# fboehm/DBSLMM

Hardware: AMD Instinct MI355X
Metric: SNPs solved/sec (whole node) + max-|Δβ| vs CPU ref, 1M SNP × 10k indiv (higher is better)
Workload: dtype f64

## Files before the change

dbslmm_amd/csrc/kernels.hip:

```cpp
#include <hip/hip_runtime.h>
#include <stdint.h>

#include "dims.hpp"

namespace {

typedef int v4i __attribute__((ext_vector_type(4)));
typedef int v16i __attribute__((ext_vector_type(16)));

constexpr int kWave = 64;
constexpr int kLdsStride = 33;

__device__ __forceinline__ void wave_sync() {
    __builtin_amdgcn_fence(__ATOMIC_RELEASE, "wavefront");
    __builtin_amdgcn_wave_barrier();
    __builtin_amdgcn_fence(__ATOMIC_ACQUIRE, "wavefront");
}

__device__ __forceinline__ int wave_sum_i32(int v) {
#pragma unroll
    for (int o = 32; o > 0; o >>= 1) v += __shfl_xor(v, o, kWave);
    return v;
}

__device__ __forceinline__ double wave_sum_f64(double v) {
#pragma unroll
    for (int o = 32; o > 0; o >>= 1) v += __shfl_xor(v, o, kWave);
    return v;
}

__device__ __forceinline__ uint32_t dose_code16(uint32_t w) {
    return 0xAAAAAAAAu - (w - ((w >> 1) & 0x55555555u));
}
__device__ __forceinline__ int64_t image_row(const int32_t* __restrict__ slot_pos, int row0, int li, int m,
                                             int32_t zrow) {
    const int32_t pos = li < m ? slot_pos[row0 + li] : -1;
    return pos < 0 ? zrow : pos;
}
typedef int v8i __attribute__((ext_vector_type(8)));
typedef float v16f __attribute__((ext_vector_type(16)));
constexpr int kE8M0Two = static_cast<int>(0x80808080u);
constexpr uint32_t kFp4Mask = 0x33333333u;
__device__ __forceinline__ v4i fp4_chunk(uint32_t w0, uint32_t w1) {
    const uint64_t t = ((static_cast<uint64_t>(w1) << 32) | w0) >> 2;
    return v4i{static_cast<int>(w0 & kFp4Mask), static_cast<int>(static_cast<uint32_t>(t) & kFp4Mask),
               static_cast<int>(w1 & kFp4Mask), static_cast<int>(static_cast<uint32_t>(t >> 32) & kFp4Mask)};
}
__device__ __forceinline__ v16f mfma_fp4(v4i a, v4i b, v16f c) {
    const v8i a8{a[0], a[1], a[2], a[3], 0, 0, 0, 0}, b8{b[0], b[1], b[2], b[3], 0, 0, 0, 0};
    return __builtin_amdgcn_mfma_scale_f32_32x32x64_f8f6f4(a8, b8, c, 4, 4, 0, kE8M0Two, 0, kE8M0Two);
}
constexpr int kE8M0Half = 0x7E7E7E7E;
__device__ __forceinline__ uint32_t raw_k44() {
    uint32_t k = 0x44444444u;
    asm volatile("" : "+v"(k));
    return k;
}
__device__ __forceinline__ v4i fp4_chunk_raw(uint32_t w0, uint32_t w1, uint32_t k44) {
    const uint64_t t = ((static_cast<uint64_t>(w1) << 32) | w0) >> 2;
    return v4i{static_cast<int>((w0 & kFp4Mask) | k44), static_cast<int>((static_cast<uint32_t>(t) & kFp4Mask) | k44),
               static_cast<int>((w1 & kFp4Mask) | k44), static_cast<int>((static_cast<uint32_t>(t >> 32) & kFp4Mask) | k44)};
}
__device__ __forceinline__ v16f mfma_fp4_raw(v4i a, v4i b, v16f c) {
    const v8i a8{a[0], a[1], a[2], a[3], 0, 0, 0, 0}, b8{b[0], b[1], b[2], b[3], 0, 0, 0, 0};
    return __builtin_amdgcn_mfma_scale_f32_32x32x64_f8f6f4(a8, b8, c, 4, 4, 0, kE8M0Half, 0, kE8M0Half);
}
__device__ __forceinline__ int gram_row(double s, int64_t kpad) { return 3 * static_cast<int>(s) - 9 * static_cast<int>(kpad); }
__device__ __forceinline__ int gram_col(double s) { return 3 * static_cast<int>(s); }
__device__ __forceinline__ int gram_exact(float t, int ri, int cj) { return static_cast<int>(t) + ri + cj; }
__device__ __forceinline__ double centre(double g, double sisj, double rn) {
    return __builtin_fma(-sisj, rn, g);
}
__device__ __forceinline__ void split_missing(uint32_t w, uint32_t& g, uint32_t& o) {
    const uint32_t m2 = w & ~(w >> 1) & 0x55555555u;
    g = dose_code16(w) & ~(3u * m2);
    o = m2 ^ 0x55555555u;
}

}

typedef unsigned int u4v __attribute__((ext_vector_type(4)));
__device__ __forceinline__ u4v load_u4(const uint8_t* p) { return *reinterpret_cast<const u4v*>(p); }
__device__ __forceinline__ u4v shift_pair(u4v x, u4v y, int d, int bs) {
    uint32_t w[8] = {x[0], x[1], x[2], x[3], y[0], y[1], y[2], y[3]};
    uint32_t o[5];
    switch (d) {
        case 0: o[0] = w[0]; o[1] = w[1]; o[2] = w[2]; o[3] = w[3]; o[4] = w[4]; break;
        case 1: o[0] = w[1]; o[1] = w[2]; o[2] = w[3]; o[3] = w[4]; o[4] = w[5]; break;
        case 2: o[0] = w[2]; o[1] = w[3]; o[2] = w[4]; o[3] = w[5]; o[4] = w[6]; break;
        default: o[0] = w[3]; o[1] = w[4]; o[2] = w[5]; o[3] = w[6]; o[4] = w[7]; break;
    }
    u4v r;
#pragma unroll
    for (int j = 0; j < 4; ++j) r[j] = __builtin_amdgcn_alignbyte(o[j + 1], o[j], static_cast<uint32_t>(bs));
    return r;
}

__device__ __forceinline__ void count_word(uint32_t word, int& sum, int& sq, int& nmiss) {
    const uint32_t lo2 = word & 0x55555555u;
    const uint32_t hi2 = (word >> 1) & 0x55555555u;
    const int n_miss = __builtin_popcount(lo2 & ~hi2);
    const int n_two = __builtin_popcount(~lo2 & ~hi2 & 0x55555555u);
    const int n_one = __builtin_popcount(~lo2 & hi2);
    nmiss += n_miss;
    sum += 2 * n_two + n_one;
    sq += 4 * n_two + n_one;
}
__device__ __forceinline__ void row_moments(int32_t n_ref, int sum, int sq, int nmiss, double& ds, double& mu,
                                            double& rsd) {
    const double dc = static_cast<double>(n_ref - nmiss);
    ds = static_cast<double>(sum);
    mu = ds / dc;
    const double css = static_cast<double>(sq) - ds * ds / dc;
    const double sd = sqrt(css / static_cast<double>(n_ref - 1));
    rsd = 1.0 / sd;
}

extern "C" __global__ __launch_bounds__(256) void dbslmm_bed_repitch(
    const uint8_t* __restrict__ bed, int32_t n_ref, int64_t bytes_per_snp, int32_t n_rows,
    uint8_t* __restrict__ img, int64_t pitch, v4i* __restrict__ tab) {
    const int lane = threadIdx.x & (kWave - 1);
    const int r = blockIdx.x * (blockDim.x / kWave) + (threadIdx.x / kWave);
    if (r > n_rows) return;
    u4v* out = reinterpret_cast<u4v*>(img + static_cast<int64_t>(r) * pitch);
    const int nq = static_cast<int>(pitch / 16);
    if (r == n_rows) {
        for (int q = lane; q < nq; q += kWave) out[q] = u4v{~0u, ~0u, ~0u, ~0u};
        if (lane == 0) tab[r] = v4i{0, 0, 0, 0};
        return;
    }
    const int64_t row_off = 3 + static_cast<int64_t>(r) * bytes_per_snp;
    const uint8_t* base = bed + (row_off & ~int64_t(15));
    const int sh = static_cast<int>(row_off & 15), dsh = sh >> 2, bsh = sh & 3;
    const int nqd = (n_ref + 63) / 64;
    int sum = 0, sq = 0, nmiss = 0;
    for (int q = lane; q < nq; q += kWave) {
        u4v g = u4v{~0u, ~0u, ~0u, ~0u};
        if (q < nqd) {
            const u4v lo = load_u4(base + 16 * static_cast<int64_t>(q));
            const u4v wv = sh ? shift_pair(lo, load_u4(base + 16 * static_cast<int64_t>(q) + 16), dsh, bsh) : lo;
#pragma unroll
            for (int j = 0; j < 4; ++j) {
                const int nv = min(16, max(0, n_ref - (64 * q + 16 * j)));
                const uint32_t keep = nv >= 16 ? ~0u : (1u << (2 * nv)) - 1u;
                g[j] = wv[j] | ~keep;
                count_word(g[j], sum, sq, nmiss);
            }
        }
        out[q] = g;
    }
    sum = wave_sum_i32(sum);
    sq = wave_sum_i32(sq);
    nmiss = wave_sum_i32(nmiss);
    if (lane == 0) tab[r] = v4i{sum, sq, nmiss, 0};
}

__device__ __forceinline__ void slot_stats_of(
    int slot, const v4i* __restrict__ tab, int32_t n_ref,
    const int32_t* __restrict__ slot_pos, const int32_t* __restrict__ slot_block, int32_t n_slots,
    double* __restrict__ S_out, double* __restrict__ mu_out, double* __restrict__ rsd_out,
    int32_t* __restrict__ block_flags) {
    if (slot >= n_slots) return;
    const int32_t pos = slot_pos ? slot_pos[slot] : slot;
    double ds = 0.0, mu = 0.0, rsd = 0.0;
    int nmiss = 0;
    if (pos >= 0) {
        const v4i e = tab[pos];
        nmiss = e[2];
        row_moments(n_ref, e[0], e[1], nmiss, ds, mu, rsd);
    }
    if (S_out) S_out[slot] = ds;
    if (mu_out) mu_out[slot] = mu;
    if (rsd_out) rsd_out[slot] = rsd;
    if (nmiss > 0 && block_flags) atomicOr(block_flags + (slot_block ? slot_block[slot] : slot), 1);
}

extern "C" __global__ __launch_bounds__(256) void dbslmm_slot_stats(
    const v4i* __restrict__ tab, int32_t n_ref,
    const int32_t* __restrict__ slot_pos, const int32_t* __restrict__ slot_block, int32_t n_slots,
    double* __restrict__ S_out, double* __restrict__ mu_out, double* __restrict__ rsd_out,
    int32_t* __restrict__ block_flags) {
    slot_stats_of(blockIdx.x * blockDim.x + threadIdx.x, tab, n_ref, slot_pos, slot_block, n_slots, S_out, mu_out,
                  rsd_out, block_flags);
}

constexpr int kFrontCopies = 4;
struct PcgFront {
    double shift[kFrontCopies];
    double* dshift;
    int32_t n;
    int32_t n_status;
    int32_t* status;
    int32_t* active;
    int32_t* next;
};
extern "C" __global__ __launch_bounds__(256) void dbslmm_pcg_front(
    const v4i* __restrict__ tab, int32_t n_ref,
    const int32_t* __restrict__ slot_pos, const int32_t* __restrict__ slot_block, int32_t n_slots,
    double* __restrict__ S_out, double* __restrict__ mu_out, double* __restrict__ rsd_out,
    int32_t* __restrict__ block_flags, PcgFront f) {
    const int t = blockIdx.x * blockDim.x + threadIdx.x, nt = gridDim.x * blockDim.x;
    for (int i = t; i < f.n_status; i += nt) f.status[i] = 0;
    if (t < f.n) f.dshift[t] = t == 0 ? f.shift[0] : t == 1 ? f.shift[1] : t == 2 ? f.shift[2] : f.shift[3];
    if (t == 0) *f.active = 0;
    if (t < 4 && f.next) f.next[t] = 0;
    slot_stats_of(t, tab, n_ref, slot_pos, slot_block, n_slots, S_out, mu_out, rsd_out, block_flags);
}

extern "C" __global__ __launch_bounds__(256) void dbslmm_snp_stats(
    const uint8_t* __restrict__ img, int32_t n_ref, int64_t pitch,
    const int32_t* __restrict__ slot_pos, int32_t n_slots,
    double* __restrict__ mu_out, double* __restrict__ rsd_out) {
    constexpr int kU = 4;
    const int lane = threadIdx.x & (kWave - 1);
    const int slot = blockIdx.x * (blockDim.x / kWave) + (threadIdx.x / kWave);
    if (slot >= n_slots) return;
    const int32_t pos = slot_pos[slot];
    if (pos < 0) {
        if (lane == 0) {
            mu_out[slot] = 0.0;
            rsd_out[slot] = 0.0;
        }
        return;
    }
    const uint8_t* base = img + static_cast<int64_t>(pos) * pitch;
    const int nqd = (n_ref + 63) / 64;
    int sum = 0, sq = 0, nmiss = 0;
    for (int q0 = 0; q0 < nqd; q0 += kWave * kU) {
        u4v wv[kU];
#pragma unroll
        for (int u = 0; u < kU; ++u) {
            const int q = q0 + kWave * u + lane;
            wv[u] = u4v{~0u, ~0u, ~0u, ~0u};
            if (q < nqd) wv[u] = load_u4(base + 16 * static_cast<int64_t>(q));
        }
#pragma unroll
        for (int u = 0; u < kU; ++u) {
#pragma unroll
            for (int j = 0; j < 4; ++j) count_word(wv[u][j], sum, sq, nmiss);
        }
    }
    sum = wave_sum_i32(sum);
    sq = wave_sum_i32(sq);
    nmiss = wave_sum_i32(nmiss);
    if (lane == 0) {
        double ds, mu, rsd;
        row_moments(n_ref, sum, sq, nmiss, ds, mu, rsd);
        mu_out[slot] = mu;
        rsd_out[slot] = rsd;
    }
}

extern "C" __global__ __launch_bounds__(256) void dbslmm_maf_arma(
    const uint8_t* __restrict__ img, int32_t n_ref, int64_t pitch,
    const int32_t* __restrict__ pos, int32_t n_rows, const double* __restrict__ mu,
    double* __restrict__ maf_out, const double* __restrict__ S, const int32_t* __restrict__ miss) {
    const int k = blockIdx.x * blockDim.x + threadIdx.x;
    if (k >= n_rows) return;
    if (miss && S && miss[k] == 0) {
        const double af = 0.5 * S[k] / static_cast<double>(n_ref);
        maf_out[k] = (1.0 - af) < af ? 1.0 - af : af;
        return;
    }
    const uint32_t* row = reinterpret_cast<const uint32_t*>(img + static_cast<int64_t>(pos ? pos[k] : k) * pitch);
    const double m = mu[k];
    double a1 = 0.0, a2 = 0.0;
    for (int32_t i0 = 0; i0 < n_ref; i0 += 16) {
        const uint32_t word = row[i0 / 16];
        const int nv = min(16, n_ref - i0);
        for (int j = 0; j < nv; j += 2) {
            const uint32_t c0 = (word >> (2 * j)) & 3u;
            a1 += c0 == 0u ? 2.0 : c0 == 2u ? 1.0 : c0 == 3u ? 0.0 : m;
            if (j + 1 < nv) {
                const uint32_t c1 = (word >> (2 * j + 2)) & 3u;
                a2 += c1 == 0u ? 2.0 : c1 == 2u ? 1.0 : c1 == 3u ? 0.0 : m;
            }
        }
    }
    const double af = 0.5 * (a1 + a2) / static_cast<double>(n_ref);
    maf_out[k] = (1.0 - af) < af ? 1.0 - af : af;
}

__device__ __forceinline__ int copy_lo(int m, int32_t tmin, int32_t tcopy) {
    return tcopy >= 0 && m >= tmin ? tcopy : 0;
}
__device__ __forceinline__ int copy_hi(int m, int32_t tmin, int32_t tcopy, int32_t ncopy) {
    return tcopy >= 0 && m >= tmin ? tcopy + 1 : ncopy;
}

__device__ __forceinline__ void gram_tile32(
    const uint8_t* __restrict__ img, int64_t kpad, const int32_t* __restrict__ slot_pos, int32_t zrow,
    int row0, int m, int ld, int64_t moff, bool missing,
    int r0, int c0, int lane, const double* __restrict__ S, const double* __restrict__ mu,
    const double* __restrict__ rsd, double n_ref_d, double pad_k, double tau, double* __restrict__ M,
    int32_t ncopy, int64_t cstride, int32_t tmin, int32_t tcopy, uint16_t* __restrict__ G16,
    int64_t g16off, int64_t g16ld) {
    const int64_t kw = kpad / 16;
    const uint32_t* pa = reinterpret_cast<const uint32_t*>(img) +
                         image_row(slot_pos, row0, r0 + (lane & 31), m, zrow) * kw + 4 * (lane >> 5);
    const uint32_t* pb = reinterpret_cast<const uint32_t*>(img) +
                         image_row(slot_pos, row0, c0 + (lane & 31), m, zrow) * kw + 4 * (lane >> 5);

    v16f acc = {0.0f};
    v16f acc_go = {0.0f}, acc_og = {0.0f}, acc_oo = {0.0f};
    if (!missing) {
        const uint32_t k44 = raw_k44();
        for (int64_t w = 0; w < kw; w += 8) {
            const v4i wa = *reinterpret_cast<const v4i*>(pa + w);
            const v4i wb = *reinterpret_cast<const v4i*>(pb + w);
#pragma unroll
            for (int q = 0; q < 2; ++q)
                acc = mfma_fp4_raw(fp4_chunk_raw(static_cast<uint32_t>(wa[2 * q]), static_cast<uint32_t>(wa[2 * q + 1]), k44),
                                   fp4_chunk_raw(static_cast<uint32_t>(wb[2 * q]), static_cast<uint32_t>(wb[2 * q + 1]), k44), acc);
        }
    } else {
        for (int64_t w = 0; w < kw; w += 8) {
          const v4i wa = *reinterpret_cast<const v4i*>(pa + w);
          const v4i wb = *reinterpret_cast<const v4i*>(pb + w);
#pragma unroll
          for (int q = 0; q < 2; ++q) {
            uint32_t ga0, oa0, ga1, oa1, gb0, ob0, gb1, ob1;
            split_missing(static_cast<uint32_t>(wa[2 * q]), ga0, oa0);
            split_missing(static_cast<uint32_t>(wa[2 * q + 1]), ga1, oa1);
            split_missing(static_cast<uint32_t>(wb[2 * q]), gb0, ob0);
            split_missing(static_cast<uint32_t>(wb[2 * q + 1]), gb1, ob1);
            const v4i ga = fp4_chunk(ga0, ga1), oa = fp4_chunk(oa0, oa1);
            const v4i gb = fp4_chunk(gb0, gb1), ob = fp4_chunk(ob0, ob1);
            acc = mfma_fp4(ga, gb, acc);
            acc_go = mfma_fp4(ga, ob, acc_go);
            acc_og = mfma_fp4(oa, gb, acc_og);
            acc_oo = mfma_fp4(oa, ob, acc_oo);
          }
        }
    }

    const int j = lane & 31;
    const int lj = c0 + j;
    const int sj = row0 + lj;
    const double Sj = lj < m ? S[sj] : 0.0;
    const int cj = gram_col(Sj);
    if (G16 && !missing) {
#pragma unroll
        for (int r = 0; r < 16; ++r) {
            const int li = r0 + (r & 3) + 8 * (r >> 2) + 4 * (lane >> 5);
            if (li < m && lj < m)
                G16[g16off + li * g16ld + lj] =
                    static_cast<uint16_t>(gram_exact(acc[r], gram_row(S[row0 + li], kpad), cj));
        }
        return;
    }
    const double muj = lj < m ? mu[sj] : 0.0;
    const double rj = lj < m ? rsd[sj] : 0.0;
    const double scale = tau / n_ref_d, rn = 1.0 / n_ref_d;
#pragma unroll
    for (int r = 0; r < 16; ++r) {
        const int i = (r & 3) + 8 * (r >> 2) + 4 * (lane >> 5);
        const int li = r0 + i;
        if (li >= m || lj >= m) continue;
        const int si = row0 + li;
        double c;
        if (!missing) {
            c = centre(static_cast<double>(gram_exact(acc[r], gram_row(S[si], kpad), cj)), S[si] * Sj, rn);
        } else {
            const double mui = mu[si];
            c = static_cast<double>(acc[r]) - muj * static_cast<double>(acc_go[r]) -
                mui * static_cast<double>(acc_og[r]) +
                mui * muj * (static_cast<double>(acc_oo[r]) - pad_k);
        }
        double v = scale * (c * rsd[si] * rj);
        if (li == lj) v += 1.0 - tau;
        const int c_lo = copy_lo(m, tmin, tcopy), c_hi = copy_hi(m, tmin, tcopy, ncopy);
        for (int cp = c_lo; cp < c_hi; ++cp) M[moff + cp * cstride + static_cast<int64_t>(li) * ld + lj] = v;
    }
}

extern "C" __global__ __launch_bounds__(256) void dbslmm_gram_i8(
    const uint8_t* __restrict__ img, int64_t kpad, const int32_t* __restrict__ slot_pos, int32_t zrow,
    const GramTile* __restrict__ tiles, int32_t n_tiles,
    const int32_t* __restrict__ blk_row0, const int32_t* __restrict__ blk_m,
    const int32_t* __restrict__ blk_ld, const int64_t* __restrict__ blk_matoff,
    const int32_t* __restrict__ block_flags,
    const double* __restrict__ S, const double* __restrict__ mu, const double* __restrict__ rsd,
    double n_ref_d, double pad_k, double tau, double* __restrict__ M,
    int32_t ncopy, int64_t cstride, int32_t tmin, int32_t tcopy, uint16_t* __restrict__ G16,
    const int64_t* __restrict__ g16off, const int32_t* __restrict__ g16ld) {
    const int lane = threadIdx.x & (kWave - 1);
    const int t = blockIdx.x * (blockDim.x / kWave) + (threadIdx.x / kWave);
    if (t >= n_tiles) return;
    const GramTile tile = tiles[t];
    const int b = tile.block;
    gram_tile32(img, kpad, slot_pos, zrow, blk_row0[b], blk_m[b], blk_ld[b], blk_matoff[b], (block_flags[b] & 1) != 0,
                kTile * tile.ti, kTile * tile.tj, lane, S, mu, rsd, n_ref_d, pad_k, tau, M, ncopy, cstride,
                tmin, tcopy, G16, G16 ? g16off[b] : 0, G16 ? g16ld[b] : 0);
}

namespace gram {
constexpr int kKS = 256;
constexpr int kRS = kKS / 2 + 16;
constexpr int kOpBytes = kGT * kRS;
constexpr int kLdsBytes = 2 * 2 * kOpBytes;
}

extern "C" __global__ __launch_bounds__(256) void dbslmm_gram_big(
    const uint8_t* __restrict__ img, int64_t kpad, const int32_t* __restrict__ slot_pos, int32_t zrow,
    const GramTile* __restrict__ tiles, int32_t n_tiles,
    const int32_t* __restrict__ blk_row0, const int32_t* __restrict__ blk_m,
    const int32_t* __restrict__ blk_ld, const int64_t* __restrict__ blk_matoff,
    const int32_t* __restrict__ block_flags,
    const double* __restrict__ S, const double* __restrict__ mu, const double* __restrict__ rsd,
    double n_ref_d, double pad_k, double tau, double* __restrict__ M,
    int32_t ncopy, int64_t cstride, int32_t tmin, int32_t tcopy, uint16_t* __restrict__ G16,
    const int64_t* __restrict__ g16off, const int32_t* __restrict__ g16ld) {
    using namespace gram;
    extern __shared__ __attribute__((aligned(16))) int8_t glds[];
    if (static_cast<int>(blockIdx.x) >= n_tiles) return;
    const GramTile tile = tiles[blockIdx.x];
    const int b = tile.block;
    if (b < 0) return;
    const int tid = threadIdx.x, lane = tid & 63, wave = tid >> 6;
    const int row0 = blk_row0[b], m = blk_m[b], ld = blk_ld[b];
    const int64_t moff = blk_matoff[b];
    const bool diag = tile.ti == tile.tj;
    if (block_flags[b] & 1) {
        for (int q = wave; q < 16; q += 4) {
            const int si = q >> 2, sj = q & 3;
            if (diag && sj > si) continue;
            const int r0 = kGT * tile.ti + 32 * si, c0 = kGT * tile.tj + 32 * sj;
            if (r0 >= m || c0 >= m) continue;
            gram_tile32(img, kpad, slot_pos, zrow, row0, m, ld, moff, true, r0, c0, lane, S, mu, rsd, n_ref_d, pad_k,
                        tau, M, ncopy, cstride, tmin, tcopy, nullptr, 0, 0);
        }
        return;
    }
    const int64_t kw = kpad / 16;
    typedef uint32_t u2 __attribute__((ext_vector_type(2)));
    const uint32_t *ga[4], *gb[4];
#pragma unroll
    for (int q = 0; q < 4; ++q) {
        const int e = q * 256 + tid, r = e >> 3, c = e & 7;
        ga[q] = reinterpret_cast<const uint32_t*>(img) + image_row(slot_pos, row0, kGT * tile.ti + r, m, zrow) * kw + 2 * c;
        gb[q] = diag ? ga[q]
                     : reinterpret_cast<const uint32_t*>(img) + image_row(slot_pos, row0, kGT * tile.tj + r, m, zrow) * kw + 2 * c;
    }
    const uint32_t k44 = raw_k44();
    u2 ra0[4], rb0[4], ra1[4], rb1[4];
    auto gload = [&](u2 (&ra)[4], u2 (&rb)[4], int st) {
        const int64_t w0 = static_cast<int64_t>(st) * (kKS / 16);
#pragma unroll
        for (int q = 0; q < 4; ++q) {
            ra[q] = *reinterpret_cast<const u2*>(ga[q] + w0);
            if (!diag) rb[q] = *reinterpret_cast<const u2*>(gb[q] + w0);
        }
    };
    auto lstore = [&](const u2 (&ra)[4], const u2 (&rb)[4], int buf) {
        int8_t* A = glds + buf * 2 * kOpBytes;
        int8_t* B = A + kOpBytes;
#pragma unroll
        for (int q = 0; q < 4; ++q) {
            const int e = q * 256 + tid, r = e >> 3, c = e & 7;
            *reinterpret_cast<v4i*>(A + r * kRS + 16 * c) = fp4_chunk_raw(ra[q][0], ra[q][1], k44);
            if (!diag) *reinterpret_cast<v4i*>(B + r * kRS + 16 * c) = fp4_chunk_raw(rb[q][0], rb[q][1], k44);
        }
    };
    const int wr = wave >> 1, wc = wave & 1;
    const bool idle = diag && wc > wr;
    v16f acc[2][2];
#pragma unroll
    for (int i = 0; i < 2; ++i)
#pragma unroll
        for (int j = 0; j < 2; ++j) acc[i][j] = v16f{0.0f};
    const int rsub = lane & 31, ksub = 16 * (lane >> 5);
    auto compute = [&](int buf) {
        if (idle) return;
        const int8_t* A = glds + buf * 2 * kOpBytes;
        const int8_t* B = diag ? A : A + kOpBytes;
        const int8_t* pa = A + (64 * wr + rsub) * kRS + ksub;
        const int8_t* pb = B + (64 * wc + rsub) * kRS + ksub;
#pragma unroll
        for (int kk = 0; kk < kKS / 2; kk += 32) {
            const v4i a0 = *reinterpret_cast<const v4i*>(pa + kk);
            const v4i a1 = *reinterpret_cast<const v4i*>(pa + 32 * kRS + kk);
            const v4i b0 = *reinterpret_cast<const v4i*>(pb + kk);
            const v4i b1 = *reinterpret_cast<const v4i*>(pb + 32 * kRS + kk);
            acc[0][0] = mfma_fp4_raw(a0, b0, acc[0][0]);
            acc[0][1] = mfma_fp4_raw(a0, b1, acc[0][1]);
            acc[1][0] = mfma_fp4_raw(a1, b0, acc[1][0]);
            acc[1][1] = mfma_fp4_raw(a1, b1, acc[1][1]);
        }
    };
    const int nst = static_cast<int>(kpad / kKS);
    gload(ra0, rb0, 0);
    lstore(ra0, rb0, 0);
    if (nst > 1) gload(ra1, rb1, 1);
    __syncthreads();
    for (int st = 0; st < nst; st += 2) {
        if (st + 2 < nst) gload(ra0, rb0, st + 2);
        compute(0);
        if (st + 1 < nst) lstore(ra1, rb1, 1);
        __syncthreads();
        if (st + 1 >= nst) break;
        if (st + 3 < nst) gload(ra1, rb1, st + 3);
        compute(1);
        if (st + 2 < nst) lstore(ra0, rb0, 0);
        __syncthreads();
    }
    if (G16) {
        int* eTerm = reinterpret_cast<int*>(glds);
        {
            const int col = tid >> 7, idx = kGT * (col ? tile.tj : tile.ti) + (tid & 127);
            const double sv = idx < m ? S[row0 + idx] : 0.0;
            eTerm[tid] = col ? gram_col(sv) : gram_row(sv, kpad);
        }
        __syncthreads();
        if (idle) return;
        const int64_t go = g16off[b], gl = g16ld[b];
#pragma unroll
        for (int sj = 0; sj < 2; ++sj) {
            const int cl = 64 * wc + 32 * sj + (lane & 31), lj = kGT * tile.tj + cl;
            if (lj >= m) continue;
            const int cj = eTerm[kGT + cl];
#pragma unroll
            for (int si = 0; si < 2; ++si)
#pragma unroll
                for (int r = 0; r < 16; ++r) {
                    const int rl = 64 * wr + 32 * si + (r & 3) + 8 * (r >> 2) + 4 * (lane >> 5);
                    const int li = kGT * tile.ti + rl;
                    if (li < m) G16[go + li * gl + lj] = static_cast<uint16_t>(gram_exact(acc[si][sj][r], eTerm[rl], cj));
                }
        }
        return;
    }
    if (idle) return;
    const double scale = tau / n_ref_d, rn = 1.0 / n_ref_d;
#pragma unroll
    for (int sj = 0; sj < 2; ++sj) {
        const int lj = kGT * tile.tj + 64 * wc + 32 * sj + (lane & 31);
        if (lj >= m) continue;
        const double Sj = S[row0 + lj], rj = rsd[row0 + lj];
#pragma unroll
        for (int si = 0; si < 2; ++si) {
#pragma unroll
            for (int r = 0; r < 16; ++r) {
                const int li = kGT * tile.ti + 64 * wr + 32 * si + (r & 3) + 8 * (r >> 2) + 4 * (lane >> 5);
                if (li >= m) continue;
                const double Si = S[row0 + li];
                const double c = centre(static_cast<double>(gram_exact(acc[si][sj][r], gram_row(Si, kpad), gram_col(Sj))),
                                        Si * Sj, rn);
                double v = scale * (c * rsd[row0 + li] * rj);
                if (li == lj) v += 1.0 - tau;
                for (int cp = copy_lo(m, tmin, tcopy); cp < copy_hi(m, tmin, tcopy, ncopy); ++cp)
                    M[moff + cp * cstride + static_cast<int64_t>(li) * ld + lj] = v;
            }
        }
    }
}

namespace gram {
constexpr int kHK = 256;
constexpr int kHLdsBytes = 4 * 2 * kHT * (kHK / 4);
static_assert(kKpadAlign == kHK, "kpad: a multiple of the stage");
}

template <int NOP, bool kFull>
__device__ __forceinline__ void gram_huge_dma_loop(const uint8_t* __restrict__ img, int64_t kw,
                                                   const int32_t* __restrict__ slot_pos, int32_t zrow,
                                                   const int64_t (&rbase)[2], const int (&svl)[2], int nst,
                                                   int8_t* lds, int wave, int lane, int wr, int wc,
                                                   uint32_t act, v16f (&acc)[2][4]) {
    typedef __attribute__((address_space(1))) const void* gptr_g;
    typedef __attribute__((address_space(3))) void* lptr_g;
    constexpr int kRowB = 64;
    constexpr int kOpB = gram::kHT * kRowB;
    constexpr int kSlotB = 2 * kOpB;
    const int dr = lane >> 2, dp = lane & 3;
    const uint32_t* gsrc[NOP][2];
#pragma unroll
    for (int op = 0; op < NOP; ++op)
#pragma unroll
        for (int h = 0; h < 2; ++h) {
            const int r = 32 * wave + 16 * h + dr;
            const int q = dp ^ ((r >> 2) & 3);
            const int32_t pos = slot_pos[rbase[op] + min(r, svl[op] - 1)];
            gsrc[op][h] = reinterpret_cast<const uint32_t*>(img) + static_cast<int64_t>(pos < 0 ? zrow : pos) * kw + 4 * q;
        }
    auto issue = [&](int st) {
        int8_t* slot = lds + (st & 3) * kSlotB;
#pragma unroll
        for (int op = 0; op < NOP; ++op)
#pragma unroll
            for (int h = 0; h < 2; ++h)
                __builtin_amdgcn_global_load_lds((gptr_g)(gsrc[op][h] + 16 * st),
                                                 (lptr_g)(slot + op * kOpB + (32 * wave + 16 * h) * kRowB), 16, 0, 0);
    };
    const uint32_t k44 = raw_k44();
    const int rsub = lane & 31, hh = lane >> 5;
    auto roff = [&](int r, int j) { return r * kRowB + 16 * ((2 * j + hh) ^ ((r >> 2) & 3)); };
    auto compute = [&](int st) {
        const int8_t* A = lds + (st & 3) * kSlotB;
        const int8_t* B = NOP == 1 ? A : A + kOpB;
        v4i ar[2][2], br[2][4];
        auto read = [&](int j) {
#pragma unroll
            for (int i = 0; i < 2; ++i) ar[j][i] = *reinterpret_cast<const v4i*>(A + roff(64 * wr + 32 * i + rsub, j));
#pragma unroll
            for (int jj = 0; jj < 4; ++jj) br[j][jj] = *reinterpret_cast<const v4i*>(B + roff(128 * wc + 32 * jj + rsub, j));
        };
        v4i av[2], bv[4];
        auto expand = [&](int j, int e) {
#pragma unroll
            for (int i = 0; i < 2; ++i)
                av[i] = fp4_chunk_raw(static_cast<uint32_t>(ar[j][i][2 * e]), static_cast<uint32_t>(ar[j][i][2 * e + 1]), k44);
#pragma unroll
            for (int jj = 0; jj < 4; ++jj)
                bv[jj] = fp4_chunk_raw(static_cast<uint32_t>(br[j][jj][2 * e]), static_cast<uint32_t>(br[j][jj][2 * e + 1]), k44);
        };
        auto mult = [&]() {
#pragma unroll
            for (int i = 0; i < 2; ++i)
#pragma unroll
                for (int jj = 0; jj < 4; ++jj)
                    if (kFull || (act & (1u << (4 * i + jj)))) acc[i][jj] = mfma_fp4_raw(av[i], bv[jj], acc[i][jj]);
        };
        read(0);
        __builtin_amdgcn_sched_barrier(0);
        expand(0, 0);
        __builtin_amdgcn_sched_barrier(0);
        read(1);
        __builtin_amdgcn_sched_barrier(0);
        mult();
        expand(0, 1);
        mult();
        __builtin_amdgcn_sched_barrier(0);
        expand(1, 0);
        mult();
        expand(1, 1);
        mult();
    };
    auto wait_stage = [&](int ahead) {
        if (ahead >= 2) {
            if constexpr (NOP == 2) asm volatile("s_waitcnt vmcnt(8)" ::: "memory");
            else asm volatile("s_waitcnt vmcnt(4)" ::: "memory");
        } else if (ahead == 1) {
            if constexpr (NOP == 2) asm volatile("s_waitcnt vmcnt(4)" ::: "memory");
            else asm volatile("s_waitcnt vmcnt(2)" ::: "memory");
        } else {
            asm volatile("s_waitcnt vmcnt(0)" ::: "memory");
        }
    };
    for (int st = 0; st < min(3, nst); ++st) issue(st);
    for (int st = 0; st < nst; ++st) {
        wait_stage(min(2, nst - 1 - st));
        __builtin_amdgcn_s_barrier();
        if (st + 3 < nst) issue(st + 3);
        compute(st);
        asm volatile("s_waitcnt lgkmcnt(0)" ::: "memory");
    }
    asm volatile("s_waitcnt vmcnt(0)" ::: "memory");
    __builtin_amdgcn_s_barrier();
}

#define GRAM_HUGE_PARAMS                                                                            \
    const uint8_t* __restrict__ img, int64_t kpad, const int32_t* __restrict__ slot_pos,           \
    int32_t zrow,                                                                                  \
    const GramTile* __restrict__ tiles, int32_t n_tiles,                                           \
    const int32_t* __restrict__ blk_row0, const int32_t* __restrict__ blk_m,                       \
    const int32_t* __restrict__ blk_ld, const int64_t* __restrict__ blk_matoff,                    \
    const int32_t* __restrict__ block_flags,                                                       \
    const double* __restrict__ S, const double* __restrict__ mu, const double* __restrict__ rsd,   \
    double n_ref_d, double pad_k, double tau, double* __restrict__ M,                              \
    int32_t ncopy, int64_t cstride, int32_t tmin, int32_t tcopy, uint16_t* __restrict__ G16,          \
    const int64_t* __restrict__ g16off, const int32_t* __restrict__ g16ld
#define GRAM_HUGE_ARGS img, kpad, slot_pos, zrow, tiles, n_tiles, blk_row0, blk_m, blk_ld, blk_matoff, block_flags, S, \
    mu, rsd, n_ref_d, pad_k, tau, M, ncopy, cstride, tmin, tcopy, G16, g16off, g16ld
__device__ __forceinline__ void gram_huge_body(GRAM_HUGE_PARAMS) {
    using namespace gram;
    extern __shared__ __attribute__((aligned(16))) int8_t hlds[];
    if (static_cast<int>(blockIdx.x) >= n_tiles) return;
    const GramTile tile = tiles[blockIdx.x];
    const int b = tile.block;
    if (b < 0) return;
    const int tid = threadIdx.x, lane = tid & 63, wave = __builtin_amdgcn_readfirstlane(tid >> 6);
    const int row0 = blk_row0[b], m = blk_m[b], ld = blk_ld[b];
    const int64_t moff = blk_matoff[b];
    const bool diag = tile.ti == tile.tj;
    if (block_flags[b] & 1) {
        for (int q = wave; q < 64; q += 8) {
            const int si = q >> 3, sj = q & 7;
            if (diag && sj > si) continue;
            const int r0 = kHT * tile.ti + 32 * si, c0 = kHT * tile.tj + 32 * sj;
            if (r0 >= m || c0 >= m) continue;
            gram_tile32(img, kpad, slot_pos, zrow, row0, m, ld, moff, true, r0, c0, lane, S, mu, rsd, n_ref_d, pad_k,
                        tau, M, ncopy, cstride, tmin, tcopy, nullptr, 0, 0);
        }
        return;
    }
    const int rv = min(kHT, m - kHT * tile.ti), cv = min(kHT, m - kHT * tile.tj);
    const int64_t kw = kpad / 16;
    auto piece_act = [&](int pr, int pc) {
        uint32_t a = 0;
#pragma unroll
        for (int i = 0; i < 2; ++i)
#pragma unroll
            for (int j = 0; j < 4; ++j) {
                const int ri = 64 * pr + 32 * i, cj = 128 * pc + 32 * j;
                if (ri < rv && cj < cv && !(diag && cj >= ri + 32)) a |= 1u << (4 * i + j);
            }
        return a;
    };
    int cnt[8];
#pragma unroll
    for (int q = 0; q < 8; ++q) cnt[q] = __builtin_popcount(piece_act(q >> 1, q & 1));
    const int rank_want = wave < 4 ? wave : 11 - wave;
    int pc_sel = 0;
#pragma unroll
    for (int q = 0; q < 8; ++q) {
        int rk = 0;
#pragma unroll
        for (int u = 0; u < 8; ++u) rk += (cnt[u] > cnt[q] || (cnt[u] == cnt[q] && u < q)) ? 1 : 0;
        if (rk == rank_want) pc_sel = q;
    }
    pc_sel = __builtin_amdgcn_readfirstlane(pc_sel);
    const int wr = pc_sel >> 1, wc = pc_sel & 1;
    uint32_t act = piece_act(wr, wc);
    act = __builtin_amdgcn_readfirstlane(act);
    const bool idle = act == 0;
    v16f acc[2][4];
#pragma unroll
    for (int i = 0; i < 2; ++i)
#pragma unroll
        for (int j = 0; j < 4; ++j) acc[i][j] = v16f{0.0f};
    {
        const int nst = static_cast<int>(kpad / kHK);
        const int64_t rbase[2] = {row0 + kHT * tile.ti, row0 + kHT * tile.tj};
        const int svl[2] = {rv, cv};
        if (diag) {
            if (act == 0xFFu) gram_huge_dma_loop<1, true>(img, kw, slot_pos, zrow, rbase, svl, nst, hlds, wave, lane, wr, wc, act, acc);
            else gram_huge_dma_loop<1, false>(img, kw, slot_pos, zrow, rbase, svl, nst, hlds, wave, lane, wr, wc, act, acc);
        } else {
            if (act == 0xFFu) gram_huge_dma_loop<2, true>(img, kw, slot_pos, zrow, rbase, svl, nst, hlds, wave, lane, wr, wc, act, acc);
            else gram_huge_dma_loop<2, false>(img, kw, slot_pos, zrow, rbase, svl, nst, hlds, wave, lane, wr, wc, act, acc);
        }
    }
    double* eRow = reinterpret_cast<double*>(hlds);
    double* eCol = eRow + 2 * kHT;
    {
        const int sop = tid >> 8, k = tid & 255, idx = kHT * (sop ? tile.tj : tile.ti) + k;
        double* e = sop ? eCol : eRow;
        e[k] = idx < m ? S[row0 + idx] : 0.0;
        e[kHT + k] = idx < m ? rsd[row0 + idx] : 0.0;
    }
    __syncthreads();
    if (idle) return;
    int cj[4];
#pragma unroll
    for (int sj = 0; sj < 4; ++sj) cj[sj] = gram_col(eCol[128 * wc + 32 * sj + (lane & 31)]);
    if (G16) {
        const int64_t go = g16off[b], gl = g16ld[b];
#pragma unroll
        for (int si = 0; si < 2; ++si)
#pragma unroll
            for (int r = 0; r < 16; ++r) {
                const int rl = 64 * wr + 32 * si + (r & 3) + 8 * (r >> 2) + 4 * (lane >> 5);
                const int li = kHT * tile.ti + rl;
                if (li >= m) continue;
                const int ri = gram_row(eRow[rl], kpad);
#pragma unroll
                for (int sj = 0; sj < 4; ++sj) {
                    const int lj = kHT * tile.tj + 128 * wc + 32 * sj + (lane & 31);
                    if (!(act & (1u << (4 * si + sj))) || lj >= m) continue;
                    G16[go + li * gl + lj] = static_cast<uint16_t>(gram_exact(acc[si][sj][r], ri, cj[sj]));
                }
            }
        return;
    }
    const double scale = tau / n_ref_d, rn = 1.0 / n_ref_d;
    double Sj[4], rj[4];
#pragma unroll
    for (int sj = 0; sj < 4; ++sj) {
        const int cl = 128 * wc + 32 * sj + (lane & 31);
        Sj[sj] = eCol[cl];
        rj[sj] = eCol[kHT + cl];
    }
#pragma unroll
    for (int si = 0; si < 2; ++si) {
#pragma unroll
        for (int r = 0; r < 16; ++r) {
            const int rl = 64 * wr + 32 * si + (r & 3) + 8 * (r >> 2) + 4 * (lane >> 5);
            const int li = kHT * tile.ti + rl;
            if (li >= m) continue;
            const double Si = eRow[rl], ri = eRow[kHT + rl];
#pragma unroll
            for (int sj = 0; sj < 4; ++sj) {
                const int lj = kHT * tile.tj + 128 * wc + 32 * sj + (lane & 31);
                if (!(act & (1u << (4 * si + sj))) || lj >= m) continue;
                const double c = centre(static_cast<double>(gram_exact(acc[si][sj][r], gram_row(Si, kpad), cj[sj])),
                                        Si * Sj[sj], rn);
                double v = scale * (c * ri * rj[sj]);
                if (li == lj) v += 1.0 - tau;
                for (int cp = copy_lo(m, tmin, tcopy); cp < copy_hi(m, tmin, tcopy, ncopy); ++cp)
                    M[moff + cp * cstride + static_cast<int64_t>(li) * ld + lj] = v;
            }
        }
    }
}

extern "C" __global__ __launch_bounds__(512) void dbslmm_gram_huge(GRAM_HUGE_PARAMS) {
    gram_huge_body(GRAM_HUGE_ARGS);
}

extern "C" __global__ __launch_bounds__(256) void dbslmm_valid_partial(
    const uint8_t* __restrict__ img, int32_t n_ref, int64_t pitch,
    const int64_t* __restrict__ ptr, const int32_t* __restrict__ pos,
    const double* __restrict__ z1, const double* __restrict__ mu, const double* __restrict__ rsd,
    double* __restrict__ partial, int32_t n_chunks, int32_t num_block) {
    __shared__ double red[256 / kWave];
    const int64_t w = static_cast<int64_t>(blockIdx.x) * blockDim.x + threadIdx.x;
    const int64_t n_words = (n_ref + 15) / 16;
    const int nv = static_cast<int>(min<int64_t>(16, n_ref - 16 * w));
    for (int b = blockIdx.y; b < num_block; b += gridDim.y) {
        double y[16];
#pragma unroll
        for (int i = 0; i < 16; ++i) y[i] = 0.0;
        if (w < n_words) {
            for (int64_t j = ptr[b]; j < ptr[b + 1]; ++j) {
#pragma clang fp contract(off)
                const uint32_t word = *reinterpret_cast<const uint32_t*>(img + static_cast<int64_t>(pos[j]) * pitch + 4 * w);
                const double m0 = mu[j], wt = z1[j] * rsd[j];
                const double t2 = (2.0 - m0) * wt, t1 = (1.0 - m0) * wt, t0 = (0.0 - m0) * wt, tm = (m0 - m0) * wt;
#pragma unroll
                for (int i = 0; i < 16; ++i) {
                    const uint32_t code = (word >> (2 * i)) & 3u;
                    const double t = code == 0 ? t2 : (code == 2 ? t1 : (code == 3 ? t0 : tm));
                    if (i < nv) y[i] += t;
                }
            }
        }
        double s = 0.0;
#pragma unroll
        for (int i = 0; i < 16; ++i) s += y[i] * y[i];
        for (int off = kWave / 2; off > 0; off >>= 1) s += __shfl_down(s, off, kWave);
        if ((threadIdx.x & (kWave - 1)) == 0) red[threadIdx.x / kWave] = s;
        __syncthreads();
        if (threadIdx.x == 0) {
            double t = 0.0;
            for (int q = 0; q < 256 / kWave; ++q) t += red[q];
            partial[static_cast<int64_t>(b) * n_chunks + blockIdx.x] = t;
        }
        __syncthreads();
    }
}

extern "C" __global__ void dbslmm_valid_reduce(const double* __restrict__ partial, int32_t n_chunks,
                                               int32_t num_block, double n_ref_d,
                                               double* __restrict__ deno) {
    const int b = blockIdx.x * blockDim.x + threadIdx.x;
    if (b >= num_block) return;
    double t = 0.0;
    for (int c = 0; c < n_chunks; ++c) t += partial[static_cast<int64_t>(b) * n_chunks + c];
    deno[b] = t / n_ref_d;
}

extern "C" __global__ void dbslmm_set_scalar(double* __restrict__ dst, double v) { *dst = v; }

extern "C" __global__ void dbslmm_debug_spin(int64_t ticks) {
    const uint64_t t0 = __builtin_amdgcn_s_memrealtime();
    while (static_cast<int64_t>(__builtin_amdgcn_s_memrealtime() - t0) < ticks) __builtin_amdgcn_s_sleep(16);
}

extern "C" __global__ __launch_bounds__(256) void dbslmm_std_columns(
    const uint8_t* __restrict__ img, int32_t n_ref, int64_t pitch,
    const int32_t* __restrict__ pos, int32_t n_rows,
    const double* __restrict__ mu, const double* __restrict__ rsd, double* __restrict__ out) {
    const int64_t idx = static_cast<int64_t>(blockIdx.x) * blockDim.x + threadIdx.x;
    if (idx >= static_cast<int64_t>(n_rows) * n_ref) return;
    const int jrow = static_cast<int>(idx / n_ref);
    const int i = static_cast<int>(idx % n_ref);
    const uint8_t byte = img[static_cast<int64_t>(pos[jrow]) * pitch + (i >> 2)];
    const int code = (byte >> (2 * (i & 3))) & 3;
    const double g = code == 0 ? 2.0 : code == 2 ? 1.0 : code == 3 ? 0.0 : mu[jrow];
    out[idx] = (g - mu[jrow]) * rsd[jrow];
}
```

dbslmm_amd/csrc/pcg.hip:

```cpp
#include <hip/hip_runtime.h>
#include <stdint.h>

namespace pcg {
constexpr int kT = 128;
constexpr int kRunMax = 8;
constexpr int kMaxNC = 4;
constexpr int kWaves = 4;
constexpr int kVS = kT + 8;
constexpr int kNDot = 5;
constexpr int kQS = 8;
constexpr int kThreads = 256;
constexpr int kFTb = 8;
constexpr int kFRows = kFTb * kT;
constexpr int kFPer = kFRows / kThreads;
__device__ __forceinline__ void chip_wide_priority() { __builtin_amdgcn_s_setprio(3); }
constexpr int wave_lds_doubles(int nc) { return 3 * nc * kVS + 4 * nc * 64; }
constexpr size_t lds_bytes(int nc) { return sizeof(double) * kWaves * wave_lds_doubles(nc); }
}

struct PcgBlk {
    int32_t blk, row0, m, ms;
    int32_t ld, Tb, Ns, sco;
    int64_t matoff, vo, po, dof;
    int64_t off16;
    int32_t nc;
    int32_t mshift;
    int32_t fused;
    int32_t pad_;
};

struct PcgArgs {
    const PcgBlk* blk;
    const uint16_t* G16;
    const double* M;
    const int32_t* flags;
    const double* S;
    const double* rsd;
    const double* z;
    const int32_t* slot_out;
    const int32_t* blk_id;
    const double* dshift;
    double *X, *R, *P, *Sv, *W;
    double* U;
    double* part;
    double* dot;
    double* qs;
    int32_t* cnv;
    int32_t* itb;
    int32_t* done;
    int32_t* active;
    int32_t* fin;
    double* beta_s;
    double* beta_l;
    int32_t* status;
    double* mir_s;
    double* mir_l;
    int32_t* mir_st;
    int32_t* mir_flag;
    int32_t run_no;
    int64_t vstride;
    int64_t ns, nl, nbk;
    double tau, rn, c0, tol, inv_sqrt_n;
    int32_t ncopy;
    int32_t run;
    int32_t seed;
};

namespace pcg {

__device__ __forceinline__ void wave_fence() {
    __builtin_amdgcn_fence(__ATOMIC_RELEASE, "wavefront");
    __builtin_amdgcn_wave_barrier();
    __builtin_amdgcn_fence(__ATOMIC_ACQUIRE, "wavefront");
}

template <int Ctrl>
__device__ __forceinline__ double dpp_mov(double v) {
    const uint64_t b = __builtin_bit_cast(uint64_t, v);
    const int lo = __builtin_amdgcn_mov_dpp(static_cast<int>(b & 0xffffffffu), Ctrl, 0xf, 0xf, false);
    const int hi = __builtin_amdgcn_mov_dpp(static_cast<int>(b >> 32), Ctrl, 0xf, 0xf, false);
    return __builtin_bit_cast(double, (static_cast<uint64_t>(static_cast<uint32_t>(hi)) << 32) | static_cast<uint32_t>(lo));
}
template <int X>
__device__ __forceinline__ uint32_t swap_xor(uint32_t x, bool up) {
    if constexpr (X == 16) {
        const auto r = __builtin_amdgcn_permlane16_swap(x, x, false, false);
        return up ? r[0] : r[1];
    } else {
        const auto r = __builtin_amdgcn_permlane32_swap(x, x, false, false);
        return up ? r[0] : r[1];
    }
}
template <int X>
__device__ __forceinline__ double lane_xor(double v) {
#ifndef PCG_NO_DPP
    if constexpr (X == 1) return dpp_mov<0xB1>(v);
    else if constexpr (X == 2) return dpp_mov<0x4E>(v);
    else if constexpr (X == 4) return dpp_mov<0x1B>(dpp_mov<0x141>(v));
    else if constexpr (X == 8) return dpp_mov<0x128>(v);
#ifndef PCG_NO_PERMLANE
    else if constexpr (X == 16 || X == 32) {
        const uint64_t b = __builtin_bit_cast(uint64_t, v);
        const bool up = (__lane_id() & X) != 0;
        const uint32_t lo = swap_xor<X>(static_cast<uint32_t>(b & 0xffffffffu), up);
        const uint32_t hi = swap_xor<X>(static_cast<uint32_t>(b >> 32), up);
        return __builtin_bit_cast(double, (static_cast<uint64_t>(hi) << 32) | lo);
    }
#endif
    else
#endif
        return __shfl_xor(v, X);
}

template <int X2, int X1, int X0>
__device__ __forceinline__ double rscatter8(const double (&v)[8], int lane) {
    const bool h2 = (lane & X2) != 0, h1 = (lane & X1) != 0, h0 = (lane & X0) != 0;
    double u[4], w[2];
#pragma unroll
    for (int q = 0; q < 4; ++q) {
        const double send = h2 ? v[q] : v[q + 4], keep = h2 ? v[q + 4] : v[q];
        u[q] = keep + lane_xor<X2>(send);
    }
#pragma unroll
    for (int q = 0; q < 2; ++q) {
        const double send = h1 ? u[q] : u[q + 2], keep = h1 ? u[q + 2] : u[q];
        w[q] = keep + lane_xor<X1>(send);
    }
    const double send = h0 ? w[0] : w[1], keep = h0 ? w[1] : w[0];
    return keep + lane_xor<X0>(send);
}

__device__ __forceinline__ double wave_sum(double v) {
    v += lane_xor<32>(v);
    v += lane_xor<16>(v);
    v += lane_xor<8>(v);
    v += lane_xor<4>(v);
    v += lane_xor<2>(v);
    v += lane_xor<1>(v);
    return v;
}



__device__ __forceinline__ double ordered_sum(const double* __restrict__ p, int64_t st, int s0, int s1, double acc) {
    for (int s = s0; s < s1; s += 8) {
        double t[8];
#pragma unroll
        for (int u = 0; u < 8; ++u) t[u] = s + u < s1 ? p[static_cast<int64_t>(s + u) * st] : 0.0;
#pragma unroll
        for (int u = 0; u < 8; ++u) acc += t[u];
    }
    return acc;
}

__device__ __forceinline__ bool on_u16(const PcgArgs& a, const PcgBlk& B) {
    return a.G16 != nullptr && (a.flags[B.blk] & 1) == 0;
}

__device__ __forceinline__ double jdiag(const PcgArgs& a, const PcgBlk& B, int i, double dc) {
    return B.mshift ? 1.0 : i < B.ms ? a.c0 + dc : a.c0;
}
__device__ __forceinline__ double col_shift(const PcgArgs& a, const PcgBlk& B, int k) {
    return a.dshift[B.mshift ? a.seed : k];
}

__device__ __forceinline__ void put_beta(const PcgArgs& a, const PcgBlk& B, int i, int k, double x, bool mono) {
    const int so = a.slot_out[B.row0 + i];
    const double bv = mono ? __builtin_nan("") : x * a.inv_sqrt_n;
    if (so >= 0) {
        a.beta_s[k * a.ns + so] = bv;
        if (a.mir_s) a.mir_s[k * a.ns + so] = bv;
    } else {
        a.beta_l[k * a.nl - 1 - so] = bv;
        if (a.mir_l) a.mir_l[k * a.nl - 1 - so] = bv;
    }
}
__device__ __forceinline__ void put_status(const PcgArgs& a, const PcgBlk& B, int k, bool mono) {
    const int st = mono ? DBSLMM_BLOCK_MONOMORPHIC
                        : a.cnv[B.sco + k] == 0 ? DBSLMM_BLOCK_NOT_CONVERGED : DBSLMM_BLOCK_OK;
    const int64_t o = k * a.nbk + a.blk_id[B.blk];
    a.status[o] = st;
    if (a.mir_st) a.mir_st[o] = st;
}

__device__ __forceinline__ double cvt_lo(uint32_t w) {
    double g;
    uint32_t t;
    asm volatile("v_and_b32 %1, 0xffff, %2\n\tv_cvt_f64_u32 %0, %1" : "=v"(g), "=&v"(t) : "v"(w));
    return g;
}
__device__ __forceinline__ double cvt_hi(uint32_t w) {
    double g;
    uint32_t t;
    asm volatile("v_lshrrev_b32 %1, 16, %2\n\tv_cvt_f64_u32 %0, %1" : "=v"(g), "=&v"(t) : "v"(w));
    return g;
}

typedef uint32_t pcg_u4 __attribute__((ext_vector_type(4)));

__device__ __forceinline__ void cvt_row(const pcg_u4& w, double (&g)[8]) {
#pragma unroll
    for (int c = 0; c < 8; ++c) g[c] = (c & 1) ? cvt_hi(w[c >> 1]) : cvt_lo(w[c >> 1]);
}

__device__ __forceinline__ __amdgpu_buffer_rsrc_t g16_rsrc(const uint16_t* base, uint32_t bytes) {
    const uint64_t gb = reinterpret_cast<uint64_t>(base);
    const uint32_t lo = static_cast<uint32_t>(__builtin_amdgcn_readfirstlane(static_cast<int>(gb & 0xffffffffu)));
    const uint32_t hi = static_cast<uint32_t>(__builtin_amdgcn_readfirstlane(static_cast<int>(gb >> 32)));
    const int nb = __builtin_amdgcn_readfirstlane(static_cast<int>(bytes));
    return __builtin_amdgcn_make_buffer_rsrc(reinterpret_cast<void*>((static_cast<uint64_t>(hi) << 32) | lo),
                                             static_cast<short>(0), nb, 0x00020000);
}
constexpr uint32_t kG16Oob = 0x80000000u;

__device__ __forceinline__ void quad_mul16(const pcg_u4 (&raw)[8], bool diagq, int lane, int nc,
                                           const double* vI, const double* vJ, double* rsum, double* csum) {
    const int rg = lane >> 3, cg = lane & 7;
#pragma unroll 1
    for (int k = 0; k < nc; ++k) {
        double vi[8], vj[8], racc[8], cacc[8];
#pragma unroll
        for (int q = 0; q < 8; ++q) {
            vi[q] = vI[k * kVS + 8 * rg + q];
            vj[q] = vJ[k * kVS + 8 * cg + q];
            racc[q] = cacc[q] = 0.0;
        }
        if (!diagq) {
#pragma unroll
            for (int r = 0; r < 8; ++r) {
                double g[8];
                cvt_row(raw[r], g);
#pragma unroll
                for (int c = 0; c < 8; ++c) {
                    racc[r] = __builtin_fma(g[c], vj[c], racc[r]);
                    cacc[c] = __builtin_fma(g[c], vi[r], cacc[c]);
                }
            }
        } else {
#pragma unroll
            for (int r = 0; r < 8; ++r) {
                double g[8];
                cvt_row(raw[r], g);
#pragma unroll
                for (int c = 0; c < 8; ++c) {
                    const int dd = 8 * (cg - rg) + c - r;
                    racc[r] = __builtin_fma(dd <= 0 ? g[c] : 0.0, vj[c], racc[r]);
                    cacc[c] = __builtin_fma(dd < 0 ? g[c] : 0.0, vi[r], cacc[c]);
                }
            }
        }
        rsum[k * 64 + lane] += rscatter8<4, 2, 1>(racc, lane);
        csum[k * 64 + lane] += rscatter8<32, 16, 8>(cacc, lane);
    }
}

__device__ __forceinline__ void quad_mul64(const double* __restrict__ base, int64_t ld, int rows_ok, int cols_ok,
                                           bool diagq, int lane, int nc, const double* vI, const double* vJ,
                                           double* rsum, double* csum) {
    const int rg = lane >> 3, cg = lane & 7;
#pragma unroll 1
    for (int k = 0; k < nc; ++k) {
        double vi[8], vj[8], racc[8], cacc[8];
#pragma unroll
        for (int q = 0; q < 8; ++q) {
            vi[q] = vI[k * kVS + 8 * rg + q];
            vj[q] = vJ[k * kVS + 8 * cg + q];
            racc[q] = cacc[q] = 0.0;
        }
#pragma unroll 1
        for (int r = 0; r < 8; ++r)
#pragma unroll
            for (int c = 0; c < 8; ++c) {
                const double g = (r < rows_ok && c < cols_ok) ? base[r * ld + c] : 0.0;
                const int dd = 8 * (cg - rg) + c - r;
                const double gr = !diagq || dd <= 0 ? g : 0.0, gc = !diagq || dd < 0 ? g : 0.0;
#pragma unroll
                for (int q = 0; q < 8; ++q)
                    if (q == r) racc[q] = __builtin_fma(gr, vj[c], racc[q]);
                cacc[c] = __builtin_fma(gc, vi[r], cacc[c]);
            }
        rsum[k * 64 + lane] += rscatter8<4, 2, 1>(racc, lane);
        csum[k * 64 + lane] += rscatter8<32, 16, 8>(cacc, lane);
    }
}

__device__ __forceinline__ void stage_v(const PcgArgs& a, const PcgBlk& B, int T, int nc, int lane, double* v) {
    for (int k = 0; k < nc; ++k) {
        const double* src = a.U + k * a.vstride + B.vo + static_cast<int64_t>(T) * kT;
        const double x0 = src[lane], x1 = src[lane + 64];
        v[k * kVS + lane] = x0;
        v[k * kVS + lane + 64] = x1;
    }
}

__device__ __forceinline__ bool quad_active(const PcgBlk& B, int I, int J, int q) {
    const int qi = q >> 1, qj = q & 1;
    return !(J == I && qj > qi) && I * kT + 64 * qi < B.m && J * kT + 64 * qj < B.m;
}
__device__ __forceinline__ bool next_quad(const PcgBlk& B, int I, int J1, int& J, int& q) {
    for (;;) {
        if (++q == 4) {
            q = 0;
            if (++J > J1) return false;
        }
        if (quad_active(B, I, J, q)) return true;
    }
}

template <bool U16>
__device__ void symv_item(const PcgArgs& a, int4 item, int lane, double* vI, double* vJb, double* rsum,
                          double* csum) {
    const PcgBlk B = a.blk[item.x];
    if (a.done[item.x] || on_u16(a, B) != U16) return;
    const int I = item.y, J0 = item.z, J1 = item.w, nc = B.nc;
    const int64_t ld16 = static_cast<int64_t>(B.Tb) * kT;
    const int rg = lane >> 3, cg = lane & 7;
    auto vj_of = [&](int J) -> double* { return J == I ? vI : vJb + ((J - J0) & 1) * nc * kVS; };
    const __amdgpu_buffer_rsrc_t g16 =
        g16_rsrc(a.G16 + B.off16 + static_cast<int64_t>(I) * kT * ld16, U16 ? static_cast<uint32_t>(kT * ld16 * 2) : 0u);
    auto load = [&](int J, int q, pcg_u4 (&raw)[8], bool none) {
        if constexpr (U16) {
            const int i0 = 64 * (q >> 1) + 8 * rg, j0 = J * kT + 64 * (q & 1) + 8 * cg;
            const bool skip = none || j0 >= B.m || (J == I && (q == 0 || q == 3) && cg > rg);
            const uint32_t o = static_cast<uint32_t>((static_cast<int64_t>(i0) * ld16 + j0) * 2);
#pragma unroll
            for (int r = 0; r < 8; ++r)
                raw[r] = __builtin_amdgcn_raw_buffer_load_b128(
                    g16, (skip || I * kT + i0 + r >= B.m) ? kG16Oob : o + static_cast<uint32_t>(r * ld16 * 2), 0, 0);
        }
    };
    auto mult = [&](int J, int q, const pcg_u4 (&raw)[8]) {
        const int qi = q >> 1, qj = q & 1;
        const bool dq = J == I && qi == qj;
        const double* vj = vj_of(J);
        double* rs = rsum + qi * nc * 64;
        double* cs = csum + qj * nc * 64;
        if constexpr (U16) {
            quad_mul16(raw, dq, lane, nc, vI + 64 * qi, vj + 64 * qj, rs, cs);
        } else {
            const int ib = I * kT + 64 * qi + 8 * rg, jb = J * kT + 64 * qj + 8 * cg;
            quad_mul64(a.M + B.matoff + static_cast<int64_t>(ib) * B.ld + jb, B.ld, B.m - ib, B.m - jb, dq,
                       lane, nc, vI + 64 * qi, vj + 64 * qj, rs, cs);
        }
    };
    auto flush = [&](int J) {
        double* dst = a.part + B.po + (static_cast<int64_t>(J) * B.Ns + I) * nc * kT;
        for (int qj = 0; qj < 2; ++qj)
            for (int k = 0; k < nc; ++k) {
                dst[k * kT + 64 * qj + 8 * cg + rg] = csum[(qj * nc + k) * 64 + lane];
                csum[(qj * nc + k) * 64 + lane] = 0.0;
            }
    };
    pcg_u4 ra[8], rb[8];
    int J = J0, q = 0;
    load(J, q, ra, false);
    stage_v(a, B, I, nc, lane, vI);
    if (J != I) stage_v(a, B, J, nc, lane, vj_of(J));
    for (int t = 0; t < 2 * nc; ++t) rsum[t * 64 + lane] = csum[t * 64 + lane] = 0.0;
    wave_fence();
    auto step = [&](pcg_u4 (&cur)[8], pcg_u4 (&nxt)[8]) -> bool {
        int Jn = J, qn = q;
        const bool more = next_quad(B, I, J1, Jn, qn);
        load(more ? Jn : J, more ? qn : q, nxt, !more);
        if (more && Jn != J && Jn != I) stage_v(a, B, Jn, nc, lane, vj_of(Jn));
        mult(J, q, cur);
        if (!more || Jn != J) flush(J);
        wave_fence();
        J = Jn;
        q = qn;
        return more;
    };
    while (step(ra, rb) && step(rb, ra)) {
    }
    double* dst = a.part + B.po + (static_cast<int64_t>(I) * B.Ns + B.Tb + J0 / a.run) * nc * kT;
    for (int qi = 0; qi < 2; ++qi)
        for (int k = 0; k < nc; ++k) dst[k * kT + 64 * qi + 8 * rg + cg] = rsum[(qi * nc + k) * 64 + lane];
}

}

extern "C" __global__ __launch_bounds__(pcg::kThreads) void dbslmm_pcg_init(PcgArgs a, const int2* __restrict__ rows,
                                                                            int32_t n_lead, int32_t skip) {
    using namespace pcg;
    __shared__ double red[kThreads / 64][kMaxNC];
    __shared__ int mono_s;
    const int g = blockIdx.x;
    const int2 it = rows[g < n_lead ? g : g + skip];
    const bool head = it.y < 0;
    const int bi = it.x, I = head ? 0 : it.y, tid = threadIdx.x;
    const PcgBlk B = a.blk[bi];
    const bool u16 = on_u16(a, B);
    const int n = a.ncopy, nc = B.nc;
    if (I == 0) {
        if (tid == 0) mono_s = 0;
        __syncthreads();
        bool mono = false;
        for (int i = tid; i < B.m; i += kThreads) mono |= !(a.rsd[B.row0 + i] < INFINITY);
        if (mono) atomicOr(&mono_s, 1);
        __syncthreads();
        if (tid < n) {
            a.cnv[B.sco + tid] = 0;
            double* q = a.qs + static_cast<int64_t>(B.sco + tid) * kQS;
            q[4] = q[5] = 1.0;
        }
        if (tid == 0) {
            a.itb[bi] = 0;
            a.fin[bi] = 0;
            const bool fz = B.fused && u16;
            a.done[bi] = mono_s ? 2 : fz ? 3 : 0;
            if (!mono_s && !fz) atomicAdd(a.active, 1);
        }
    }
    if (head) return;
    const int r = tid & (kT - 1), h = tid >> 7, i = I * kT + r;
    const bool in = i < B.m;
    double sv[kMaxNC];
#pragma unroll
    for (int k = 0; k < kMaxNC; ++k) sv[k] = 0.0;
    for (int c = h; c < n; c += 2) {
        const int64_t o = c * a.vstride + B.vo + i;
        const double rhs = in ? a.z[B.row0 + i] : 0.0;
        a.X[o] = 0.0;
        a.P[o] = 0.0;
        if (c < nc) {
            a.Sv[o] = 0.0;
            a.W[o] = 0.0;
            a.R[o] = rhs;
            double uv = 0.0;
            if (in) {
                uv = rhs / jdiag(a, B, i, col_shift(a, B, c));
                if (u16) uv *= a.rsd[B.row0 + i];
            }
            a.U[o] = uv;
        }
    }
#pragma unroll
    for (int k = 0; k < kMaxNC; ++k)
        if (k < nc && (k & 1) == h && in && u16) {
            const double rhs = a.z[B.row0 + i];
            sv[k] = a.S[B.row0 + i] * a.rsd[B.row0 + i] * (rhs / jdiag(a, B, i, col_shift(a, B, k)));
        }
#pragma unroll
    for (int k = 0; k < kMaxNC; ++k) sv[k] = wave_sum(sv[k]);
    if ((tid & 63) == 0)
#pragma unroll
        for (int k = 0; k < kMaxNC; ++k) red[tid >> 6][k] = sv[k];
    __syncthreads();
    if (tid < nc) {
        const int hk = tid & 1;
        a.dot[B.dof + (static_cast<int64_t>(I) * kNDot + 4) * n + tid] = red[2 * hk][tid] + red[2 * hk + 1][tid];
    }
}

template <bool U16>
__device__ __forceinline__ void symv_body(const PcgArgs& a, const int4* __restrict__ items, int32_t n_items) {
    using namespace pcg;
    extern __shared__ double vlds[];
    chip_wide_priority();
    const int wave = threadIdx.x >> 6, lane = threadIdx.x & 63;
    const int e = blockIdx.x * kWaves + wave;
    if (e >= n_items) return;
    const int nc = a.ncopy;
    double* w = vlds + wave * wave_lds_doubles(nc);
    symv_item<U16>(a, items[e], lane, w, w + nc * kVS, w + 3 * nc * kVS, w + 3 * nc * kVS + 2 * nc * 64);
}
#ifndef PCG_SYMV_WAVES
#define PCG_SYMV_WAVES 2
#endif
extern "C" __global__ __launch_bounds__(pcg::kThreads) __attribute__((amdgpu_waves_per_eu(PCG_SYMV_WAVES, 8)))
void dbslmm_pcg_symv16(PcgArgs a, const int4* __restrict__ items, int32_t n_items) {
    symv_body<true>(a, items, n_items);
}
extern "C" __global__ __launch_bounds__(pcg::kThreads)
void dbslmm_pcg_symv64(PcgArgs a, const int4* __restrict__ items, int32_t n_items) {
    symv_body<false>(a, items, n_items);
}

extern "C" __global__ __launch_bounds__(pcg::kThreads) void dbslmm_pcg_rows(PcgArgs a, const int2* __restrict__ rows) {
    using namespace pcg;
    __shared__ double red[kThreads / 64][kMaxNC][4];
    __shared__ double sig[kMaxNC];
    chip_wide_priority();
    const int2 it = rows[blockIdx.x];
    const int bi = it.x, I = it.y, tid = threadIdx.x;
    if (a.done[bi]) return;
    const PcgBlk B = a.blk[bi];
    const bool u16 = on_u16(a, B);
    const int n = a.ncopy, nc = B.nc;
    if (tid < nc)
        sig[tid] = ordered_sum(a.dot + B.dof + 4 * n + tid, kNDot * n, 0, B.Tb, 0.0);
    __syncthreads();
    const int r = tid & (kT - 1), h = tid >> 7, i = I * kT + r;
    const bool in = i < B.m;
    const double Si = in ? a.S[B.row0 + i] : 0.0, ri = in ? a.rsd[B.row0 + i] : 0.0;
    const int nrun = (I + a.run) / a.run;
    double dv[kMaxNC][4];
#pragma unroll
    for (int k = 0; k < kMaxNC; ++k)
#pragma unroll
        for (int f = 0; f < 4; ++f) dv[k][f] = 0.0;
#pragma unroll
    for (int k = 0; k < kMaxNC; ++k) {
        if (k >= n || (k & 1) != h) continue;
        const int64_t o = k * a.vstride + B.vo + i;
        if (k < nc) {
            const double* pp = a.part + B.po + static_cast<int64_t>(I) * B.Ns * nc * kT + k * kT + r;
            double y = ordered_sum(pp, nc * kT, I, B.Tb, 0.0);
            y = ordered_sum(pp, nc * kT, B.Tb, B.Tb + nrun, y);
            const double dc = col_shift(a, B, k);
            const double rv = a.R[o];
            const double u = in ? rv / jdiag(a, B, i, dc) : 0.0;
            const double sh = i < B.ms ? dc : 0.0;
            double w = 0.0;
            if (in) {
                if (u16) w = a.tau * a.rn * ri * __builtin_fma(-Si, sig[k] * a.rn, y) + (1.0 - a.tau + sh) * u;
                else w = y + sh * u;
            }
            a.W[o] = w;
            dv[k][0] = rv * u;
            dv[k][1] = w * u;
            dv[k][2] = rv * rv;
        }
        const double xv = a.X[o];
        dv[k][3] = xv * xv;
    }
#pragma unroll
    for (int k = 0; k < kMaxNC; ++k)
#pragma unroll
        for (int f = 0; f < 4; ++f) dv[k][f] = wave_sum(dv[k][f]);
    if ((tid & 63) == 0)
#pragma unroll
        for (int k = 0; k < kMaxNC; ++k)
#pragma unroll
            for (int f = 0; f < 4; ++f) red[tid >> 6][k][f] = dv[k][f];
    __syncthreads();
    if (tid < 4 * n) {
        const int k = tid >> 2, f = tid & 3, hk = k & 1;
        if (f == 3 || k < nc)
            a.dot[B.dof + (static_cast<int64_t>(I) * kNDot + f) * n + k] = red[2 * hk][k][f] + red[2 * hk + 1][k][f];
    }
    if (I == 0 && tid == 0) a.itb[bi] += 1;
}

extern "C" __global__ __launch_bounds__(pcg::kThreads) void dbslmm_pcg_update(PcgArgs a, const int2* __restrict__ rows) {
    using namespace pcg;
    __shared__ double tot[kMaxNC][4];
    __shared__ double coef[kMaxNC][3];
    __shared__ double seedc[2];
    __shared__ int run_s[kMaxNC];
    __shared__ double red[kThreads / 64][kMaxNC];
    chip_wide_priority();
    const int2 it = rows[blockIdx.x];
    const int bi = it.x, I = it.y, tid = threadIdx.x;
    if (a.done[bi]) return;
    const PcgBlk B = a.blk[bi];
    const bool u16 = on_u16(a, B);
    const int n = a.ncopy, nc = B.nc;
    const int itn = a.itb[bi] - 1;
    const int par = itn & 1;
    if (tid < 4 * n) {
        const int k = tid >> 2, f = tid & 3;
        tot[k][f] = (f == 3 || k < nc) ? ordered_sum(a.dot + B.dof + f * n + k, kNDot * n, 0, B.Tb, 0.0) : 0.0;
    }
    __syncthreads();
    if (B.mshift) {
        if (tid == 0) {
            const double gam = tot[0][0], del = tot[0][1];
            const double* q = a.qs + static_cast<int64_t>(B.sco) * kQS;
            double al, be = 0.0;
            if (itn == 0) {
                al = gam / del;
            } else {
                be = gam / q[2 * par];
                al = gam / (del - be * gam / q[2 * par + 1]);
            }
            seedc[0] = al;
            seedc[1] = be;
        }
        __syncthreads();
        if (tid < n) {
            const int c = tid;
            double* q = a.qs + static_cast<int64_t>(B.sco + c) * kQS;
            const double al = seedc[0], be = seedc[1];
            const double zk = q[4 + 2 * par], zk1 = q[4 + 2 * par + 1];
            const double rr = tot[0][2] * zk * zk, xx = tot[c][3];
            const double t = a.tol * (a.dshift[c] + 1.0 - a.tau);
            const bool conv = a.cnv[B.sco + c] != 0 || rr == 0.0 || rr <= t * t * xx;
            const double e = a.dshift[c] - a.dshift[a.seed];
            const double cp = itn == 0 ? 0.0 : al * be / a.qs[static_cast<int64_t>(B.sco) * kQS + 2 * par + 1];
            const double zn = zk * zk1 / ((1.0 + cp + al * e) * zk1 - cp * zk);
            coef[c][0] = al * zn / zk;
            coef[c][1] = zk1 != 0.0 ? (zk / zk1) * (zk / zk1) * be : 0.0;
            coef[c][2] = zk;
            run_s[c] = conv ? 0 : 1;
            if (I == 0) {
                if (conv && a.cnv[B.sco + c] == 0) a.cnv[B.sco + c] = itn + 1;
                q[4 + 2 * (par ^ 1)] = zn;
                q[4 + 2 * (par ^ 1) + 1] = zk;
            }
        }
        __syncthreads();
        if (I == 0 && tid == 0) {
            double* q = a.qs + static_cast<int64_t>(B.sco) * kQS;
            q[2 * (par ^ 1)] = tot[0][0];
            q[2 * (par ^ 1) + 1] = seedc[0];
        }
    } else {
        if (tid < n) {
            const int k = tid;
            const double gam = tot[k][0], del = tot[k][1], rr = tot[k][2], xx = tot[k][3];
            const double lam = B.ms == B.m ? a.dshift[k] + 1.0 - a.tau : 1.0 - a.tau;
            const double t = a.tol * lam;
            const bool conv = a.cnv[B.sco + k] != 0 || rr == 0.0 || rr <= t * t * xx;
            double al = 0.0, be = 0.0;
            if (!conv) {
                double* q = a.qs + static_cast<int64_t>(B.sco + k) * kQS;
                if (itn == 0) {
                    al = gam / del;
                } else {
                    be = gam / q[2 * par];
                    al = gam / (del - be * gam / q[2 * par + 1]);
                }
                if (I == 0) {
                    q[2 * (par ^ 1)] = gam;
                    q[2 * (par ^ 1) + 1] = al;
                }
            } else if (I == 0 && a.cnv[B.sco + k] == 0) {
                a.cnv[B.sco + k] = itn + 1;
            }
            coef[k][0] = al;
            coef[k][1] = be;
            coef[k][2] = 1.0;
            run_s[k] = conv ? 0 : 1;
        }
        __syncthreads();
    }
    int running = 0;
    for (int k = 0; k < n; ++k) running += run_s[k];
    if (running == 0) {
        const int r = tid & (kT - 1), h = tid >> 7, i = I * kT + r;
        if (i < B.m)
            for (int k = h; k < n; k += 2) put_beta(a, B, i, k, a.X[k * a.vstride + B.vo + i], false);
        if (I == 0 && tid < n) put_status(a, B, tid, false);
        __syncthreads();
        if (tid == 0 &&
            __hip_atomic_fetch_add(a.fin + bi, 1, __ATOMIC_ACQ_REL, __HIP_MEMORY_SCOPE_AGENT) == B.Tb - 1) {
            a.done[bi] = 1;
            atomicSub(a.active, 1);
            if (a.mir_flag)
                for (int c = 0; c < n; ++c)
                    __hip_atomic_store(a.mir_flag + static_cast<int64_t>(bi) * n + c, a.run_no, __ATOMIC_RELEASE,
                                       __HIP_MEMORY_SCOPE_SYSTEM);
        }
        return;
    }
    const int r = tid & (kT - 1), h = tid >> 7, i = I * kT + r;
    const bool in = i < B.m;
    double sv[kMaxNC];
#pragma unroll
    for (int k = 0; k < kMaxNC; ++k) sv[k] = 0.0;
    if (B.mshift) {
        if (in) {
            const int64_t o0 = B.vo + i;
            const double rv = a.R[o0];
#pragma unroll
            for (int c = 0; c < kMaxNC; ++c) {
                if (c >= n || (c & 1) != h || !run_s[c]) continue;
                const int64_t o = c * a.vstride + o0;
                const double p = __builtin_fma(coef[c][1], a.P[o], coef[c][2] * rv);
                a.P[o] = p;
                a.X[o] = __builtin_fma(coef[c][0], p, a.X[o]);
            }
            if (h == 0) {
                const double al = seedc[0], be = seedc[1];
                const double sn = __builtin_fma(be, a.Sv[o0], a.W[o0]);
                const double rn = __builtin_fma(-al, sn, rv);
                a.Sv[o0] = sn;
                a.R[o0] = rn;
                a.U[o0] = u16 ? rn * a.rsd[B.row0 + i] : rn;
                if (u16) sv[0] = a.S[B.row0 + i] * a.rsd[B.row0 + i] * rn;
            }
        }
    } else {
#pragma unroll
        for (int k = 0; k < kMaxNC; ++k) {
            if (k >= n || (k & 1) != h || !run_s[k] || !in) continue;
            const int64_t o = k * a.vstride + B.vo + i;
            const double al = coef[k][0], be = coef[k][1];
            const double dg = jdiag(a, B, i, a.dshift[k]);
            const double u = a.R[o] / dg;
            const double p = __builtin_fma(be, a.P[o], u);
            const double s = __builtin_fma(be, a.Sv[o], a.W[o]);
            const double x = __builtin_fma(al, p, a.X[o]);
            const double rn = __builtin_fma(-al, s, a.R[o]);
            a.P[o] = p;
            a.Sv[o] = s;
            a.X[o] = x;
            a.R[o] = rn;
            a.U[o] = u16 ? (rn / dg) * a.rsd[B.row0 + i] : rn / dg;
            if (u16) sv[k] = a.S[B.row0 + i] * a.rsd[B.row0 + i] * (rn / dg);
        }
    }
#pragma unroll
    for (int k = 0; k < kMaxNC; ++k) sv[k] = wave_sum(sv[k]);
    if ((tid & 63) == 0)
#pragma unroll
        for (int k = 0; k < kMaxNC; ++k) red[tid >> 6][k] = sv[k];
    __syncthreads();
    if (tid < nc && (B.mshift || run_s[tid])) {
        const int hk = tid & 1;
        a.dot[B.dof + (static_cast<int64_t>(I) * kNDot + 4) * n + tid] = red[2 * hk][tid] + red[2 * hk + 1][tid];
    }
}

namespace pcg {
template <int N>
__device__ __forceinline__ void block_sum(double (&v)[N], double* red, int tid) {
#pragma unroll
    for (int k = 0; k < N; ++k) v[k] = wave_sum(v[k]);
    __syncthreads();
    if ((tid & 63) == 0)
#pragma unroll
        for (int k = 0; k < N; ++k) red[(tid >> 6) * N + k] = v[k];
    __syncthreads();
#pragma unroll
    for (int k = 0; k < N; ++k) v[k] = ((red[k] + red[N + k]) + red[2 * N + k]) + red[3 * N + k];
}
constexpr size_t block_lds_bytes(int n) {
    return sizeof(double) * ((5 + 2 * n) * kFRows + 4 * (3 + kMaxNC) + 12 + 3 * kMaxNC + 4);
}
}

__device__ __forceinline__ void pcg_block_solve(const PcgArgs& a, int bi, int cc, int32_t maxit) {
    using namespace pcg;
    extern __shared__ double blds[];
    double* yw = blds;
    double* Ul = blds + 4 * kFRows;
    const int n = a.ncopy;
    double* Xl = Ul + kFRows;
    double* Pl = Xl + n * kFRows;
    double* red = Pl + n * kFRows;
    if (a.done[bi] != 3) return;
    const PcgBlk B = a.blk[bi];
    const int tid = threadIdx.x, lane = tid & 63;
    const int wave = __builtin_amdgcn_readfirstlane(tid >> 6);
    const int m = B.m, Tb = B.Tb;
    const bool msh = cc < 0;
    const int nx = msh ? n : 1;
    const double dc = msh ? col_shift(a, B, 0) : a.dshift[cc];
    const int Q = (m + 63) / 64;
    const int nq = Q * (Q + 1) / 2;
    const int nw = (nq + 3 - wave) >> 2;
    const int64_t ld16 = static_cast<int64_t>(Tb) * kT;
    const int rg = lane >> 3, cg = lane & 7;
    struct QPos {
        int t, qi, qj;
    };
    auto adv = [](QPos& p, int k) {
        p.t += k;
        p.qj += k;
        while (p.qj > p.qi) {
            p.qj -= p.qi + 1;
            ++p.qi;
        }
    };
    QPos first{0, 0, 0};
    adv(first, wave);
    QPos second = first;
    adv(second, 4);
    const __amdgpu_buffer_rsrc_t g16 = g16_rsrc(a.G16 + B.off16, static_cast<uint32_t>(ld16 * ld16 * 2));
    auto load = [&](const QPos& p, pcg_u4 (&raw)[8]) {
        const int r0 = 64 * p.qi + 8 * rg, c0 = 64 * p.qj + 8 * cg;
        const bool skip = p.t >= nq || c0 >= m || (p.qi == p.qj && cg > rg);
        const uint32_t o = static_cast<uint32_t>((r0 * static_cast<int>(ld16) + c0) * 2);
#pragma unroll
        for (int rr = 0; rr < 8; ++rr)
            raw[rr] = __builtin_amdgcn_raw_buffer_load_b128(
                g16, (skip || r0 + rr >= m) ? kG16Oob : o + static_cast<uint32_t>(rr * ld16 * 2), 0, 0);
    };
    pcg_u4 ra[8], rb[8], rc[8];
    load(first, ra);
    load(second, rb);
    double r[kFPer], sv[kFPer], wv[kFPer], Sr[kFPer], Rr[kFPer], sg[1] = {0.0};
#pragma unroll
    for (int q = 0; q < kFPer; ++q) {
        const int i = tid + kThreads * q;
        const bool in = i < m;
        r[q] = in ? a.z[B.row0 + i] : 0.0;
        Sr[q] = in ? a.S[B.row0 + i] : 0.0;
        Rr[q] = in ? a.rsd[B.row0 + i] : 0.0;
        sv[q] = wv[q] = 0.0;
        double u = 0.0;
        if (in) {
            u = (r[q] / jdiag(a, B, i, dc)) * Rr[q];
            sg[0] += Sr[q] * u;
        }
        Ul[i] = u;
        for (int w = 0; w < 4; ++w) yw[w * kFRows + i] = 0.0;
        for (int c = 0; c < nx; ++c) Xl[c * kFRows + i] = Pl[c * kFRows + i] = 0.0;
    }
    block_sum(sg, red, tid);
    double sig = sg[0];
    auto mult = [&](const QPos& p, const pcg_u4 (&raw)[8]) {
        const int qi = p.qi, qj = p.qj;
        const bool dq = qi == qj;
        double vi[8], vj[8], racc[8], cacc[8];
#pragma unroll
        for (int q = 0; q < 8; ++q) {
            vi[q] = Ul[64 * qi + 8 * rg + q];
            vj[q] = Ul[64 * qj + 8 * cg + q];
            racc[q] = cacc[q] = 0.0;
        }
        if (!dq) {
#pragma unroll
            for (int rr = 0; rr < 8; ++rr) {
                double g[8];
                cvt_row(raw[rr], g);
#pragma unroll
                for (int c = 0; c < 8; ++c) {
                    racc[rr] = __builtin_fma(g[c], vj[c], racc[rr]);
                    cacc[c] = __builtin_fma(g[c], vi[rr], cacc[c]);
                }
            }
        } else {
#pragma unroll
            for (int rr = 0; rr < 8; ++rr) {
                double g[8];
                cvt_row(raw[rr], g);
#pragma unroll
                for (int c = 0; c < 8; ++c) {
                    const int dd = 8 * (cg - rg) + c - rr;
                    racc[rr] = __builtin_fma(dd <= 0 ? g[c] : 0.0, vj[c], racc[rr]);
                    cacc[c] = __builtin_fma(dd < 0 ? g[c] : 0.0, vi[rr], cacc[c]);
                }
            }
        }
        double* y = yw + wave * kFRows;
        const int ri = 64 * qi + 8 * rg + cg, ci = 64 * qj + 8 * cg + rg;
        y[ri] += rscatter8<4, 2, 1>(racc, lane);
        wave_fence();
        y[ci] += rscatter8<32, 16, 8>(cacc, lane);
    };
    double* st = red + 4 * (3 + kMaxNC);
    int* flag = reinterpret_cast<int*>(st + 12 + 3 * kMaxNC);
    if (tid == 0) {
        for (int c = 0; c < kMaxNC; ++c) {
            st[4 + c] = st[8 + c] = 1.0;
            flag[c] = c >= n;
        }
    }
    int it = 0;
    for (; it < maxit; ++it) {
        __syncthreads();
        {
            QPos pm = first, pl = second;
            adv(pl, 4);
            int s = 0;
            for (; s + 3 < nw; s += 3) {
                load(pl, rc);
                adv(pl, 4);
                mult(pm, ra);
                adv(pm, 4);
                load(pl, ra);
                adv(pl, 4);
                mult(pm, rb);
                adv(pm, 4);
                load(pl, rb);
                adv(pl, 4);
                mult(pm, rc);
                adv(pm, 4);
            }
            if (nw > 0) {
                const int rem = nw - s;
                load(pl, rc);
                mult(pm, ra);
                adv(pm, 4);
                load(first, ra);
                if (rem >= 2) {
                    mult(pm, rb);
                    adv(pm, 4);
                }
                load(second, rb);
                if (rem >= 3) mult(pm, rc);
            }
        }
        __syncthreads();
        double d[3 + kMaxNC];
#pragma unroll
        for (int k = 0; k < 3 + kMaxNC; ++k) d[k] = 0.0;
#pragma unroll
        for (int q = 0; q < kFPer; ++q) {
            const int i = tid + kThreads * q;
            double y = 0.0;
            if (i < Tb * kT) {
                y = ((yw[i] + yw[kFRows + i]) + yw[2 * kFRows + i]) + yw[3 * kFRows + i];
#pragma unroll
                for (int w = 0; w < 4; ++w) yw[w * kFRows + i] = 0.0;
            }
            if (i < m) {
                const double Si = Sr[q], ri = Rr[q];
                const double u = r[q] / jdiag(a, B, i, dc);
                const double sh = i < B.ms ? dc : 0.0;
                const double w = a.tau * a.rn * ri * __builtin_fma(-Si, sig * a.rn, y) + (1.0 - a.tau + sh) * u;
                wv[q] = w;
                d[0] += r[q] * u;
                d[1] += w * u;
                d[2] += r[q] * r[q];
                for (int c = 0; c < nx; ++c) {
                    const double xv = Xl[c * kFRows + i];
                    d[3 + c] += xv * xv;
                }
            }
        }
        block_sum(d, red, tid);
        if (tid == 0) {
            const double gam = d[0], del = d[1], rr = d[2];
            double al, be = 0.0;
            if (it == 0) {
                al = gam / del;
            } else {
                be = gam / st[0];
                al = gam / (del - be * gam / st[1]);
            }
            int running = 0;
            if (msh) {
                const double cp = it == 0 ? 0.0 : al * be / st[1];
                for (int c = 0; c < n; ++c) {
                    const double zk = st[4 + c], zk1 = st[8 + c];
                    const double t = a.tol * (a.dshift[c] + 1.0 - a.tau);
                    const double rrc = rr * zk * zk;
                    if (!flag[c] && (rrc == 0.0 || rrc <= t * t * d[3 + c])) {
                        flag[c] = 1;
                        a.cnv[B.sco + c] = it + 1;
                    }
                    const double e = a.dshift[c] - a.dshift[a.seed];
                    const double zn = zk * zk1 / ((1.0 + cp + al * e) * zk1 - cp * zk);
                    st[12 + 3 * c] = al * zn / zk;
                    st[12 + 3 * c + 1] = zk1 != 0.0 ? (zk / zk1) * (zk / zk1) * be : 0.0;
                    st[12 + 3 * c + 2] = zk;
                    st[8 + c] = zk;
                    st[4 + c] = zn;
                    running += flag[c] ? 0 : 1;
                }
            } else {
                const double lam = B.ms == B.m ? dc + 1.0 - a.tau : 1.0 - a.tau;
                const double t = a.tol * lam;
                if (rr == 0.0 || rr <= t * t * d[3]) {
                    flag[0] = 1;
                    a.cnv[B.sco + cc] = it + 1;
                }
                running = flag[0] ? 0 : 1;
            }
            st[0] = gam;
            st[1] = al;
            st[2] = al;
            st[3] = be;
            flag[kMaxNC] = running;
        }
        __syncthreads();
        if (flag[kMaxNC] == 0) break;
        const double al = st[2], be = st[3];
        double sg2[1] = {0.0};
#pragma unroll
        for (int q = 0; q < kFPer; ++q) {
            const int i = tid + kThreads * q;
            if (i >= m) continue;
            const double rsd_i = Rr[q];
            double rn;
            if (msh) {
                for (int c = 0; c < n; ++c) {
                    if (flag[c]) continue;
                    const int o = c * kFRows + i;
                    const double pv = __builtin_fma(st[12 + 3 * c + 1], Pl[o], st[12 + 3 * c + 2] * r[q]);
                    Pl[o] = pv;
                    Xl[o] = __builtin_fma(st[12 + 3 * c], pv, Xl[o]);
                }
                const double sn = __builtin_fma(be, sv[q], wv[q]);
                rn = __builtin_fma(-al, sn, r[q]);
                sv[q] = sn;
                r[q] = rn;
                Ul[i] = rn * rsd_i;
            } else {
                const double dg = jdiag(a, B, i, dc);
                const double u = r[q] / dg;
                const double pv = __builtin_fma(be, Pl[i], u);
                const double sn = __builtin_fma(be, sv[q], wv[q]);
                Pl[i] = pv;
                Xl[i] = __builtin_fma(al, pv, Xl[i]);
                rn = __builtin_fma(-al, sn, r[q]);
                sv[q] = sn;
                r[q] = rn;
                Ul[i] = (rn / dg) * rsd_i;
            }
            sg2[0] += Sr[q] * Ul[i];
        }
        block_sum(sg2, red, tid);
        sig = sg2[0];
    }
#pragma unroll
    for (int q = 0; q < kFPer; ++q) {
        const int i = tid + kThreads * q;
        if (i < m)
            for (int c = 0; c < nx; ++c) put_beta(a, B, i, msh ? c : cc, Xl[c * kFRows + i], false);
    }
    if (tid == 0) {
        atomicMax(a.itb + bi, it + (it < maxit ? 1 : 0));
        for (int c = 0; c < nx; ++c) put_status(a, B, msh ? c : cc, false);
    }
    if (a.mir_flag) {
        __syncthreads();
        if (tid == 0)
            for (int c = 0; c < nx; ++c)
                __hip_atomic_store(a.mir_flag + static_cast<int64_t>(bi) * n + (msh ? c : cc), a.run_no,
                                   __ATOMIC_RELEASE, __HIP_MEMORY_SCOPE_SYSTEM);
    }
}

extern "C" __global__ __launch_bounds__(pcg::kThreads)
__attribute__((amdgpu_waves_per_eu(1, 8), amdgpu_num_vgpr(312)))
void dbslmm_pcg_block(PcgArgs a, const int2* __restrict__ list, int32_t n_list, int32_t* __restrict__ next,
                      int32_t maxit) {
    __shared__ int e_s;
    for (;;) {
        __syncthreads();
        if (threadIdx.x == 0) e_s = atomicAdd(next, 1);
        __syncthreads();
        const int e = e_s;
        if (e >= n_list) break;
        pcg_block_solve(a, list[e].x, list[e].y, maxit);
    }
}

extern "C" __global__ __launch_bounds__(pcg::kThreads) void dbslmm_pcg_final(PcgArgs a, const int2* __restrict__ rows) {
    using namespace pcg;
    const int2 it = rows[blockIdx.x];
    const int bi = it.x, I = it.y, tid = threadIdx.x;
    const int done = a.done[bi];
    if (done == 3 || done == 1) return;
    const PcgBlk B = a.blk[bi];
    const bool mono = done == 2;
    const int r = tid & (kT - 1), h = tid >> 7, i = I * kT + r;
    if (i < B.m)
        for (int k = h; k < a.ncopy; k += 2) put_beta(a, B, i, k, a.X[k * a.vstride + B.vo + i], mono);
    if (I == 0 && tid < a.ncopy) put_status(a, B, tid, mono);
}
```

dbslmm_amd/csrc/plan_state.hpp:

```cpp
#pragma once

namespace {
enum Ev {
    kEvStart,
    kEvStatsEnd,
    kEvGramEnd,
    kEvLargeEnd,
    kEvSmallBegin,
    kEvSmallEnd,
    kEvTiledBegin,
    kEvEnd,
    kEvTiledEnd,
    kEvLeadGramBegin,
    kEvLeadGramEnd,
    kEvRestEnd,
    kEvCount,
    kEvPcgBlockBegin = kEvLargeEnd,
    kEvPcgBlockEnd = kEvSmallBegin,
};
static_assert(sizeof(v4i) == kRowEntryBytes, "one row-table entry");
struct PanelImage {
    std::shared_ptr<uint8_t> mem;
    int64_t pitch = 0;
    int32_t n_rows = 0, n_ref = 0;
    int64_t image_bytes() const { return (static_cast<int64_t>(n_rows) + 1) * pitch; }
    const v4i* rows() const { return reinterpret_cast<const v4i*>(mem.get() + image_bytes()); }
};
std::mutex g_capture_mu;
}

struct dbslmm_ctx {
    int device = 0;
    hipStream_t stream = nullptr;
    hipStream_t stream2 = nullptr;
    hipStream_t stream3 = nullptr;
    hipStream_t stream4 = nullptr, stream5 = nullptr;
    hipEvent_t fork = nullptr, join = nullptr, join3 = nullptr, fork2 = nullptr, join4 = nullptr;
    int n_cu = 256;
    std::string err;
    const uint8_t* bed_host = nullptr;
    int64_t bed_host_len = 0;
    std::shared_ptr<uint8_t> bed_cache;
    PanelImage img_cache;
    bool bed_from_fd = false;
    std::vector<dbslmm_ctx*> subs;
    std::thread setup;
    std::mutex setup_mu;
    bool setup_ok = true;
};
struct dbslmm_plan;
struct DeviceShard {
    dbslmm_plan* plan = nullptr;
    dbslmm_ctx* ctx = nullptr;
    dbslmm_ctx* own_ctx = nullptr;
    int device_index = 0;
    int copy = -1;
    std::vector<int32_t> blocks;
    std::vector<int64_t> s_idx, l_idx;
    std::vector<int> run_copies;
    std::vector<double> dl_s, dl_l;
    std::vector<int32_t> dl_st;
};
struct dbslmm_mplan {
    std::vector<DeviceShard> shards;
    int32_t n_copies = 1;
    bool partial = false;
    std::vector<int32_t> unit_device;
};

struct PlanOptions {
    int32_t solver = 0;
    double pcg_tol = 1e-12;
    int32_t pcg_maxit = 1000;
    bool pcg_fused = true;
    int32_t pcg_block_wgs = 0;
    bool stream_out = true;
    int32_t h2f_mode = 0;
    double cheb_tol = 1e-9;
    bool cheb_fused = false;
    bool h2f_cg = false;
    int32_t debug_delay_us = 0;
    int32_t debug_stop = 0;
};

struct LastRun {
    bool ran = false;
    bool stopped = false;
    double sigma_run = 0.0;
    int32_t var_copy = 0;
    int32_t score_copies = 0;
    bool score_stale = false;
    bool pcg_ran = false;
    bool pcg_pending_var = false;
    int32_t cheb_base = -1;
    bool cheb_pending_var = false;
    bool cg_ran = false;
    double cheb_iters = 0;
    double cheb_bytes = 0;
};

struct PcgState {
    bool g16 = false;
    int32_t m_blocks = -1;
    uint16_t* d_G16 = nullptr;
    int64_t* d_off16 = nullptr;
    int32_t* d_ld16 = nullptr;
    std::vector<int64_t> h_off16;
    int32_t n = 0;
    PcgBlk* d_pblk = nullptr;
    int4* d_pitem = nullptr;
    int2* d_prow = nullptr;
    int32_t n_pblk = 0, n_pitem = 0, n_prow = 0;
    int32_t n_pitem_chip = 0, n_prow_chip = 0;
    int32_t n_phead = 0;
    bool trim = false;
    int32_t run = pcg::kRunMax;
    int2* d_pflist = nullptr;
    int32_t* d_pfnext = nullptr;
    int32_t n_pflist = 0;
    std::vector<char> h_pfused;
    std::vector<int32_t> h_pnseq;
    bool join = false;
    double *d_pvec = nullptr, *d_ppart = nullptr, *d_pdot = nullptr, *d_pqs = nullptr;
    int32_t *d_pcnv = nullptr, *d_pitb = nullptr, *d_pdone = nullptr, *d_pact = nullptr, *d_pfin = nullptr;
    int64_t vstride = 0;
    PinnedBuf mon;
    int32_t it = 0;
    int32_t need = -1;
    int32_t iters_max = 0;
    bool pending = false;
    std::vector<double> h_pmat, h_ppart;
    std::vector<char> h_pmiss;
    double cbytes = 0.0, pbytes = 0.0, fbytes = 0.0;
    PcgArgs args{};
    int32_t* h_mon() const { return mon.get<int32_t>(); }
};

struct StreamOut {
    bool want = false;
    bool active = false;
    PinnedBuf mir{hipHostMallocMapped | hipHostMallocCoherent}, mflag{hipHostMallocMapped | hipHostMallocCoherent};
    int32_t n = 0;
    int32_t run = 0;
    EventList ev;
    std::vector<int2> h_pfpairs;
    std::vector<int32_t> done;
};

struct FactorState {
    int32_t* d_tlist = nullptr;
    std::vector<TLaunch> tl_multi;
    int32_t* d_tlist_multi = nullptr;
    int32_t multi_n = 0;
    GraphExecs graph_multi;
    GraphExecs graph_copy;
    GraphExecs graph_rest;
    EventList tev, tev_rest;
    int32_t *d_tri_f = nullptr, *d_tri_b = nullptr, *d_foff = nullptr, *d_tflags = nullptr, *d_tb = nullptr;
    int32_t* d_tepi = nullptr;
    int32_t* d_cheb_items = nullptr;
    int32_t n_cheb_items = 0, cheb_items_K = -1;
    int32_t trsv_epoch = 0;
    double h2f_tol = 1e-9;
    double* d_cgrec = nullptr;
    int32_t* d_cgconv = nullptr;
    int32_t* d_cgit = nullptr;
    int32_t* d_tcheb_blocks = nullptr;
    bool trsv_pending = false;
    bool trsv_failed = false;
    unsigned long long* d_stamps = nullptr;
    double* d_cheb = nullptr;
    double* d_coef = nullptr;
    int32_t coef_cap = 0;
    std::vector<double> h_coef;
    void drop_graphs() {
        graph_multi.reset();
        graph_copy.reset();
        graph_rest.reset();
    }
};

struct Timing {
    bool timing = false;
    EventList ev{hipEventDefault};
    std::vector<char> run_route;
    int runs_pending = 0;
    double ms_acc[DBSLMM_K_COUNT] = {0, 0, 0, 0, 0, 0};
    int32_t ms_runs = 0;
    hipEvent_t pcg_ev_end = nullptr;
};

struct dbslmm_plan : PlanLayout::Kept {
    dbslmm_ctx* ctx = nullptr;
    dbslmm_mplan* mp = nullptr;
    int32_t n_ref = 0, n_obs = 0, num_block = 0;
    double sigma_s = 0.0, tau = 0.8;
    int64_t bed_len = 0;
    PlanOptions opt;
    LastRun last;
    int64_t n_runs = 0;
    bool force_factor = false;
    DevBufs bufs;
    PanelImage img;
    const uint8_t* d_img = nullptr;
    int32_t *d_slot_pos = nullptr, *d_slot_block = nullptr, *d_slot_out = nullptr;
    double *d_z = nullptr, *d_S = nullptr, *d_mu = nullptr, *d_rsd = nullptr, *d_y = nullptr;
    int32_t *d_flags = nullptr, *d_status = nullptr, *d_order = nullptr, *d_blk_id = nullptr;
    int32_t *d_row0 = nullptr, *d_m = nullptr, *d_ms = nullptr, *d_ld = nullptr;
    int64_t* d_matoff = nullptr;
    GramTile* d_tiles = nullptr;
    GramTile* d_btiles = nullptr;
    GramTile* d_htiles = nullptr;
    double* d_M = nullptr;
    double *d_beta_s = nullptr, *d_beta_l = nullptr;
    double* d_dshift = nullptr;
    int32_t n_copies = 0;
    int32_t m_copies = 0;
    int64_t nbk = 1;
    PinnedBuf pin;
    EventList dl_ev;
    PcgState pcg;
    StreamOut so;
    FactorState fac;
    Timing tm;
};

struct CopyView {
    double *M, *dshift, *y, *beta_s, *beta_l;
    int32_t* status;
};
static CopyView copy_view(const dbslmm_plan* p, int64_t c) {
    return {p->d_M + c * p->M_elems,   p->d_dshift + c,           p->d_y + c * p->n_slots,
            p->d_beta_s + c * p->n_s,  p->d_beta_l + c * p->n_l,  p->d_status + c * p->nbk};
}
template <class A, class = void>
struct HasLd : std::false_type {};
template <class A>
struct HasLd<A, std::void_t<decltype(std::declval<A&>().ld)>> : std::true_type {};
template <class A>
static void set_plan_args(A& a, const dbslmm_plan* p, double inv_sqrt_n) {
    a.row0 = p->d_row0;
    a.m = p->d_m;
    a.ms = p->d_ms;
    a.blk_id = p->d_blk_id;
    a.slot_out = p->d_slot_out;
    if constexpr (HasLd<A>::value) {
        a.ld = p->d_ld;
        a.matoff = p->d_matoff;
    }
    a.inv_sqrt_n = inv_sqrt_n;
    a.beta_s = p->d_beta_s;
    a.beta_l = p->d_beta_l;
    a.ns_stride = p->n_s;
    a.nl_stride = p->n_l;
}

#define HIP_TRY(ctx, expr)                                                               \
    do {                                                                                 \
        hipError_t e_ = (expr);                                                          \
        if (e_ != hipSuccess) {                                                          \
            (ctx)->err = std::string(#expr) + " (" __FILE_NAME__ ":" + std::to_string(__LINE__) + "): " + \
                         hipGetErrorString(e_);                                          \
            return DBSLMM_E_HIP;                                                         \
        }                                                                                \
    } while (0)

#define ARG_CHECK(ctx, cond, msg)                   \
    do {                                            \
        if (!(cond)) {                              \
            (ctx)->err = msg;                       \
            return DBSLMM_E_ARG;                    \
        }                                           \
    } while (0)

static int mp_create(dbslmm_ctx* ctx, const dbslmm_problem* pr, dbslmm_plan** out);
static void mp_destroy(dbslmm_plan* p);
static int mp_download(dbslmm_plan* p, int copy, double* beta_s, double* beta_l, int32_t* block_status);
static int mp_download_all(dbslmm_plan* p, int n, double* beta_s, double* beta_l, int32_t* block_status);
static int mp_run(dbslmm_plan* p, const double* sigmas, int n, bool wait);
static int mp_sync(dbslmm_plan* p);
static int mp_block_iters(dbslmm_plan* p, int32_t* iters);
static int mp_variance(dbslmm_plan* p, const dbslmm_test_panel* tp, double* diags, int32_t* n_test_out);
static int mp_score(dbslmm_plan* p, const dbslmm_test_panel* tp, const dbslmm_score_args* args, int32_t n_copies,
                    double* scores, int32_t* dropped, int32_t* n_test_out, double* gpu_ms);
static int mp_bed_maf(dbslmm_ctx* ctx, const uint8_t* bed, int32_t n_ref, int64_t n_snp, double* maf);
#define ON_FIRST_DEVICE(ctx, call)                                       \
    do {                                                                 \
        if (!(ctx)->subs.empty()) {                                      \
            dbslmm_ctx* ctx0_ = (ctx)->subs[0];                          \
            const int rc_ = call;                                        \
            if (rc_ != DBSLMM_OK) (ctx)->err = ctx0_->err;               \
            return rc_;                                                  \
        }                                                                \
    } while (0)
```

dbslmm_amd/csrc/route_pcg.hip:

```cpp

constexpr double kPcgDmin = 2.0;
static bool pcg_eligible(const dbslmm_plan* p, const double* sigmas, int n) {
    if (p->force_factor || p->opt.solver == 1 || p->n_nonempty == 0 || p->opt.debug_stop) return false;
    if (!(p->tau > 0.0 && p->tau <= 1.0) || (p->tau >= 1.0 && p->has_large)) return false;
    if (p->opt.solver == 2) return true;
    for (int c = 0; c < n; ++c)
        if (1.0 / (sigmas[c] * static_cast<double>(p->n_obs)) < kPcgDmin) return false;
    return true;
}
static bool pcg_route(const dbslmm_plan* p, const double* sigmas, int n) {
    return n <= pcg::kMaxNC && pcg_eligible(p, sigmas, n);
}

static int pcg_layout(dbslmm_plan* p, int n) {
    dbslmm_ctx* ctx = p->ctx;
    if (p->pcg.g16 && !p->pcg.d_G16) {
        std::vector<int64_t> off;
        std::vector<int32_t> ldv;
        int64_t o = 0;
        for (int b = 0; b < p->n_nonempty; ++b) {
            const int64_t l = (p->h_m[b] + pcg::kT - 1) / pcg::kT * pcg::kT;
            off.push_back(o);
            ldv.push_back(static_cast<int32_t>(l));
            o += l * l;
        }
        const size_t e = static_cast<size_t>(o) + 256;
        HIP_TRY(ctx, p->bufs.zeroed(&p->pcg.d_G16, e, ctx->stream));
        HIP_TRY(ctx, p->bufs.upload(&p->pcg.d_off16, off, ctx->stream));
        HIP_TRY(ctx, p->bufs.upload(&p->pcg.d_ld16, ldv, ctx->stream));
        p->pcg.h_off16 = off;
    }
    HIP_TRY(ctx, p->pcg.mon.reserve((1 + std::max(1, p->n_nonempty)) * sizeof(int32_t)));
    if (p->pcg.n == n) return DBSLMM_OK;
    HIP_TRY(ctx, hipStreamSynchronize(ctx->stream));
    DevBufs& B = p->bufs;
    B.release_all(p->pcg.d_pblk, p->pcg.d_pitem, p->pcg.d_prow, p->pcg.d_pvec, p->pcg.d_ppart, p->pcg.d_pdot, p->pcg.d_pqs, p->pcg.d_pcnv,
                  p->pcg.d_pitb, p->pcg.d_pdone, p->pcg.d_pact, p->pcg.d_pflist, p->pcg.d_pfin);
    p->pcg.n = 0;
    p->pcg.trim = false;
    using namespace pcg;
    std::vector<PcgBlk> blk;
    std::vector<int2> flist;
    std::vector<double> mat, part;
    std::vector<int4> items;
    std::vector<int2> rows;
    int64_t vo = 0, po = 0, dof = 0;
    int32_t sco = 0;
    const double esz = p->pcg.g16 ? 2.0 : 8.0;
    int run = 1;
    p->pcg.run = run;
    for (int b = 0; b < p->n_nonempty; ++b) {
        const int32_t m = p->h_m[b], Tb = (m + kT - 1) / kT, nrun = (Tb + run - 1) / run;
        const bool msh = n > 1 && p->h_ms[b] == m;
        const int32_t nc = msh ? 1 : n;
        const bool fused = p->opt.pcg_fused && Tb <= kFTb && !p->pcg.h_off16.empty();
        PcgBlk k{b, p->h_row0[b], m, p->h_ms[b], p->h_ld[b], Tb, Tb + nrun, sco, p->h_matoff[b], vo, po, dof,
                 p->pcg.h_off16.empty() ? 0 : p->pcg.h_off16[b], nc, msh ? 1 : 0, fused ? 1 : 0, 0};
        if (fused) {
            const int32_t bi = static_cast<int32_t>(blk.size());
            if (nc == 1) flist.push_back(int2{bi, msh ? -1 : 0});
            else for (int c = 0; c < nc; ++c) flist.push_back(int2{bi, c});
        }
        const int bi = static_cast<int>(blk.size());
        blk.push_back(k);
        vo += static_cast<int64_t>(Tb) * kT;
        po += static_cast<int64_t>(Tb) * k.Ns * nc * kT;
        dof += static_cast<int64_t>(Tb) * kNDot * n;
        sco += n;
        for (int I = 0; I < Tb; ++I) {
            rows.push_back(int2{bi, I});
            for (int J0 = 0; J0 <= I; J0 += run) items.push_back(int4{bi, I, J0, std::min(I, J0 + run - 1)});
        }
        mat.push_back(0.5 * m * (m + 1.0) * esz);
        double runs = 0.0;
        for (int I = 0; I < Tb; ++I) runs += I / run + 1;
        part.push_back(fused ? 0.0 : 2.0 * 8.0 * nc * kT * (0.5 * Tb * (Tb + 1.0) + runs));
    }
    std::stable_sort(items.begin(), items.end(), [&](const int4& x, const int4& y) {
        return blk[x.x].fused != blk[y.x].fused ? blk[x.x].fused < blk[y.x].fused : blk[x.x].Tb > blk[y.x].Tb;
    });
    std::stable_sort(flist.begin(), flist.end(), [&](const int2& x, const int2& y) { return blk[x.x].Tb > blk[y.x].Tb; });
    std::stable_sort(rows.begin(), rows.end(), [&](const int2& x, const int2& y) { return blk[x.x].fused < blk[y.x].fused; });
    p->pcg.n_prow_chip = p->pcg.n_pitem_chip = 0;
    for (const int2& r : rows) p->pcg.n_prow_chip += blk[r.x].fused ? 0 : 1;
    for (const int4& e : items) p->pcg.n_pitem_chip += blk[e.x].fused ? 0 : 1;
    p->pcg.h_pfused.assign(blk.size(), 0);
    p->pcg.h_pnseq.assign(blk.size(), 0);
    for (const int2& f : flist) {
        p->pcg.h_pfused[f.x] = 1;
        p->pcg.h_pnseq[f.x] += 1;
    }
    p->pcg.n_pflist = static_cast<int32_t>(flist.size());
    p->so.h_pfpairs.clear();
    for (const int2& f : flist)
        for (int c = f.y < 0 ? 0 : f.y; c < (f.y < 0 ? n : f.y + 1); ++c) p->so.h_pfpairs.push_back(int2{f.x, c});
    for (int b = 0; b < static_cast<int>(blk.size()); ++b)
        if (!blk[b].fused)
            for (int c = 0; c < n; ++c) p->so.h_pfpairs.push_back(int2{b, c});
    if (!flist.empty()) HIP_TRY(ctx, B.upload(&p->pcg.d_pflist, flist, ctx->stream));
    if (!flist.empty() && !p->pcg.d_pfnext) HIP_TRY(ctx, B.alloc(&p->pcg.d_pfnext, 4));
    p->pcg.n_pblk = static_cast<int32_t>(blk.size());
    p->pcg.n_pitem = static_cast<int32_t>(items.size());
    p->pcg.n_prow = static_cast<int32_t>(rows.size());
    for (int b = 0; b < static_cast<int>(blk.size()); ++b)
        if (blk[b].fused) rows.push_back(int2{b, -1});
    p->pcg.n_phead = static_cast<int32_t>(rows.size()) - p->pcg.n_prow;
    p->pcg.vstride = vo;
    p->pcg.h_pmat = mat;
    p->pcg.h_ppart = part;
    HIP_TRY(ctx, B.upload(&p->pcg.d_pblk, blk, ctx->stream));
    HIP_TRY(ctx, B.upload(&p->pcg.d_pitem, items, ctx->stream));
    HIP_TRY(ctx, B.upload(&p->pcg.d_prow, rows, ctx->stream));
    HIP_TRY(ctx, B.alloc(&p->pcg.d_pvec, 6 * n * vo));
    HIP_TRY(ctx, B.alloc(&p->pcg.d_ppart, po));
    HIP_TRY(ctx, B.alloc(&p->pcg.d_pdot, dof));
    HIP_TRY(ctx, B.alloc(&p->pcg.d_pqs, static_cast<size_t>(std::max<int32_t>(1, sco)) * pcg::kQS));
    HIP_TRY(ctx, B.alloc(&p->pcg.d_pcnv, sco));
    HIP_TRY(ctx, B.alloc(&p->pcg.d_pitb, p->pcg.n_pblk));
    HIP_TRY(ctx, B.alloc(&p->pcg.d_pdone, p->pcg.n_pblk));
    HIP_TRY(ctx, B.alloc(&p->pcg.d_pact, 1));
    HIP_TRY(ctx, B.alloc(&p->pcg.d_pfin, p->pcg.n_pblk));
    p->pcg.n = n;
    return DBSLMM_OK;
}

static int pcg_first_chunk(const dbslmm_plan* p, const double* sigmas, int n) {
    if (p->pcg.need >= 0) return std::min(p->pcg.need, p->opt.pcg_maxit);
    double dmin = INFINITY;
    for (int c = 0; c < n; ++c) dmin = std::min(dmin, 1.0 / (sigmas[c] * static_cast<double>(p->n_obs)));
    const double kap = 1.0 + 12.0 / std::max(1e-3, dmin + 1.0 - p->tau);
    const double q = (std::sqrt(kap) - 1.0) / (std::sqrt(kap) + 1.0);
    const int k = static_cast<int>(std::ceil(std::log(2.0 / p->opt.pcg_tol) / -std::log(q))) + 2 + (p->has_large ? 4 : 0);
    return std::clamp(k, 1, p->opt.pcg_maxit);
}

static int pcg_iters(dbslmm_plan* p, int K) {
    dbslmm_ctx* ctx = p->ctx;
    hipStream_t s = ctx->stream;
    for (int k = 0; k < K; ++k) {
        const int32_t ni = p->pcg.trim ? p->pcg.n_pitem_chip : p->pcg.n_pitem, nr = p->pcg.trim ? p->pcg.n_prow_chip : p->pcg.n_prow;
        if (ni == 0 && nr == 0) continue;
        const dim3 g((std::max(1, ni) + pcg::kWaves - 1) / pcg::kWaves);
        if (p->pcg.g16)
            hipLaunchKernelGGL(dbslmm_pcg_symv16, g, dim3(pcg::kThreads), pcg::lds_bytes(p->pcg.n), s, p->pcg.args,
                               p->pcg.d_pitem, ni);
        if (!p->pcg.g16 || p->pcg.m_blocks != 0)
            hipLaunchKernelGGL(dbslmm_pcg_symv64, g, dim3(pcg::kThreads), pcg::lds_bytes(p->pcg.n), s, p->pcg.args,
                               p->pcg.d_pitem, ni);
        hipLaunchKernelGGL(dbslmm_pcg_rows, dim3(std::max(1, nr)), dim3(pcg::kThreads), 0, s, p->pcg.args, p->pcg.d_prow);
        hipLaunchKernelGGL(dbslmm_pcg_update, dim3(std::max(1, nr)), dim3(pcg::kThreads), 0, s, p->pcg.args, p->pcg.d_prow);
    }
    HIP_TRY(ctx, hipGetLastError());
    p->pcg.it += K;
    if (p->pcg.join) {
        HIP_TRY(ctx, hipStreamWaitEvent(s, ctx->join, 0));
        p->pcg.join = false;
    }
    hipLaunchKernelGGL(dbslmm_pcg_final, dim3(p->pcg.n_prow), dim3(pcg::kThreads), 0, s, p->pcg.args, p->pcg.d_prow);
    HIP_TRY(ctx, hipGetLastError());
    HIP_TRY(ctx, hipMemcpyAsync(p->pcg.h_mon(), p->pcg.d_pact, sizeof(int32_t), hipMemcpyDeviceToHost, s));
    HIP_TRY(ctx, hipMemcpyAsync(p->pcg.h_mon() + 1, p->pcg.d_pitb, p->pcg.n_pblk * sizeof(int32_t), hipMemcpyDeviceToHost, s));
    if (p->tm.pcg_ev_end) HIP_TRY(ctx, hipEventRecord(p->tm.pcg_ev_end, s));
    if (p->so.active) HIP_TRY(ctx, hipEventRecord(p->so.ev[0], s));
    return DBSLMM_OK;
}

static int pcg_check(dbslmm_plan* p) {
    dbslmm_ctx* ctx = p->ctx;
    if (p->pcg.pending) {
        HIP_TRY(ctx, hipSetDevice(ctx->device));
        HIP_TRY(ctx, hipStreamSynchronize(ctx->stream));
        int32_t need = 0;
        for (int b = 0; b < p->pcg.n_pblk; ++b)
            if (p->pcg.h_pfused.empty() || !p->pcg.h_pfused[b]) need = std::max(need, p->pcg.h_mon()[1 + b]);
        if (p->pcg.h_mon()[0] <= 0 || p->pcg.it >= p->opt.pcg_maxit) {
            p->pcg.pending = false;
            p->pcg.need = p->pcg.h_mon()[0] <= 0 ? need : p->opt.pcg_maxit;
            p->pcg.iters_max = 0;
            for (int b = 0; b < p->pcg.n_pblk; ++b) p->pcg.iters_max = std::max(p->pcg.iters_max, p->pcg.h_mon()[1 + b]);
            if (p->pcg.m_blocks < 0) {
                std::vector<int32_t> fl(std::max(1, p->n_nonempty));
                HIP_TRY(ctx, hipMemcpy(fl.data(), p->d_flags, fl.size() * sizeof(int32_t), hipMemcpyDeviceToHost));
                p->pcg.m_blocks = 0;
                p->pcg.h_pmiss.assign(p->pcg.n_pblk, 0);
                for (int b = 0; b < p->n_nonempty; ++b) {
                    p->pcg.m_blocks += fl[b] & 1;
                    if (b < p->pcg.n_pblk) p->pcg.h_pmiss[b] = fl[b] & 1;
                }
            }
            p->pcg.trim = true;
            for (int b = 0; b < p->pcg.n_pblk && b < static_cast<int>(p->pcg.h_pfused.size()); ++b)
                if (p->pcg.h_pfused[b] && p->pcg.h_pmiss[b]) p->pcg.trim = false;
            p->pcg.cbytes = p->pcg.pbytes = p->pcg.fbytes = 0.0;
            for (int b = 0; b < p->pcg.n_pblk && b < static_cast<int>(p->pcg.h_pmat.size()); ++b) {
                const double it = p->pcg.h_mon()[1 + b];
                const bool miss = !p->pcg.h_pmiss.empty() && p->pcg.h_pmiss[b];
                const double mb = p->pcg.h_pmat[b] * (miss && p->pcg.g16 ? 4.0 : 1.0);
                if (!p->pcg.h_pfused.empty() && p->pcg.h_pfused[b] && !miss) {
                    p->pcg.fbytes += it * mb * p->pcg.h_pnseq[b];
                } else {
                    p->pcg.cbytes += it * mb;
                    p->pcg.pbytes += it * p->pcg.h_ppart[b];
                }
            }
            return DBSLMM_OK;
        }
        const int K = std::min(std::max(4, p->pcg.it / 4), p->opt.pcg_maxit - p->pcg.it);
        if (const int rc = pcg_iters(p, K)) return rc;
    }
    return DBSLMM_OK;
}

static int pcg_finish(dbslmm_plan* p) {
    while (p->pcg.pending)
        if (const int rc = pcg_check(p)) return rc;
    return DBSLMM_OK;
}

static int so_prepare(dbslmm_plan* p, int n) {
    dbslmm_ctx* ctx = p->ctx;
    const size_t bytes = static_cast<size_t>(n) * (p->n_s + p->n_l) * sizeof(double) +
                         static_cast<size_t>(n) * p->nbk * sizeof(int32_t);
    HIP_TRY(ctx, p->so.mir.reserve(bytes));
    const size_t nf = static_cast<size_t>(std::max(1, p->n_nonempty)) * pcg::kMaxNC;
    const bool fresh = !p->so.mflag.get();
    HIP_TRY(ctx, p->so.mflag.reserve(nf * sizeof(int32_t)));
    HIP_TRY(ctx, p->so.ev.grow(1));
    if (fresh || p->so.run == INT32_MAX) {
        memset(p->so.mflag.get(), 0, nf * sizeof(int32_t));
        p->so.done.assign(nf, 0);
        p->so.run = 0;
    }
    p->so.run++;
    p->so.n = n;
    return DBSLMM_OK;
}

static int run_pcg(dbslmm_plan* p, const double* sigmas, int n) {
    dbslmm_ctx* ctx = p->ctx;
    auto diag_error = [](const char* when) {
#ifdef DBSLMM_DIAG
        const hipError_t e = hipGetLastError();
        if (e != hipSuccess) fprintf(stderr, "run_pcg: %s: %s\n", when, hipGetErrorString(e));
#endif
    };
    diag_error("stale error on entry");
    if (const int rc = ensure_copies(p, n, 1)) return rc;
    diag_error("error after ensure_copies");
    if (const int rc = pcg_layout(p, n)) return rc;
    diag_error("error after pcg_layout");
    p->so.active = p->so.want && p->opt.stream_out;
    if (p->so.active)
        if (const int rc = so_prepare(p, n)) return rc;
    hipStream_t s = ctx->stream;
    hipEvent_t* ev = nullptr;
    if (const int rc = open_timed_run(p, true, &ev)) return rc;
    p->tm.pcg_ev_end = ev ? ev[kEvEnd] : nullptr;
    p->fac.trsv_failed = false;
    if (ev) HIP_TRY(ctx, hipEventRecord(ev[kEvStart], s));
    static_assert(pcg::kMaxNC <= kFrontCopies, "PcgFront carries every copy's shift");
    PcgFront fr{};
    for (int c = 0; c < n; ++c) fr.shift[c] = 1.0 / (sigmas[c] * static_cast<double>(p->n_obs));
    fr.dshift = p->d_dshift;
    fr.n = n;
    fr.n_status = static_cast<int32_t>(n * p->nbk);
    fr.status = p->d_status;
    fr.active = p->pcg.d_pact;
    fr.next = p->pcg.n_pflist > 0 ? p->pcg.d_pfnext : nullptr;
    hipLaunchKernelGGL(dbslmm_pcg_front, dim3(std::max(1, (p->n_slots + 255) / 256)), dim3(256), 0, s, p->img.rows(),
                       p->n_ref, p->d_slot_pos, p->d_slot_block, p->n_slots, p->d_S, p->d_mu, p->d_rsd, p->d_flags, fr);
    HIP_TRY(ctx, hipGetLastError());
    if (ev) HIP_TRY(ctx, hipEventRecord(ev[kEvStatsEnd], s));
    uint16_t* g16 = p->pcg.g16 ? p->pcg.d_G16 : nullptr;
    const double nrd = static_cast<double>(p->n_ref);
    const GramOut go{1, INT32_MAX, -1, g16, p->pcg.d_off16, p->pcg.d_ld16};
    HIP_TRY(ctx, launch_gram(p, s, kGramHuge, p->d_htiles, p->n_htiles, go));
    HIP_TRY(ctx, launch_gram(p, s, kGramI8, p->d_tiles, p->n_tiles, go));
    HIP_TRY(ctx, launch_gram(p, s, kGramBig, p->d_btiles, p->n_btiles, go));
    if (ev) HIP_TRY(ctx, hipEventRecord(ev[kEvGramEnd], s));
    PcgArgs a{};
    a.blk = p->pcg.d_pblk;
    a.G16 = g16;
    a.M = p->d_M;
    a.flags = p->d_flags;
    a.S = p->d_S;
    a.rsd = p->d_rsd;
    a.z = p->d_z;
    a.slot_out = p->d_slot_out;
    a.blk_id = p->d_blk_id;
    a.dshift = p->d_dshift;
    const int64_t vs = static_cast<int64_t>(n) * p->pcg.vstride;
    a.X = p->pcg.d_pvec;
    a.R = a.X + vs;
    a.P = a.R + vs;
    a.Sv = a.P + vs;
    a.W = a.Sv + vs;
    a.U = a.W + vs;
    a.part = p->pcg.d_ppart;
    a.dot = p->pcg.d_pdot;
    a.qs = p->pcg.d_pqs;
    a.cnv = p->pcg.d_pcnv;
    a.itb = p->pcg.d_pitb;
    a.done = p->pcg.d_pdone;
    a.active = p->pcg.d_pact;
    a.fin = p->pcg.d_pfin;
    a.beta_s = p->d_beta_s;
    a.beta_l = p->d_beta_l;
    a.status = p->d_status;
    if (p->so.active) {
        void *dm = nullptr, *df = nullptr;
        HIP_TRY(ctx, hipHostGetDevicePointer(&dm, p->so.mir.get(), 0));
        HIP_TRY(ctx, hipHostGetDevicePointer(&df, p->so.mflag.get<int32_t>(), 0));
        a.mir_s = static_cast<double*>(dm);
        a.mir_l = a.mir_s + static_cast<int64_t>(n) * p->n_s;
        a.mir_st = reinterpret_cast<int32_t*>(a.mir_l + static_cast<int64_t>(n) * p->n_l);
        a.mir_flag = static_cast<int32_t*>(df);
        a.run_no = p->so.run;
    }
    a.vstride = p->pcg.vstride;
    a.ns = p->n_s;
    a.nl = p->n_l;
    a.nbk = p->nbk;
    a.tau = p->tau;
    a.rn = 1.0 / nrd;
    a.c0 = p->tau * (nrd - 1.0) / nrd + 1.0 - p->tau;
    a.tol = p->opt.pcg_tol;
    a.inv_sqrt_n = 1.0 / std::sqrt(static_cast<double>(p->n_obs));
    a.ncopy = n;
    a.run = p->pcg.run;
    for (int c = 1; c < n; ++c)
        if (sigmas[c] > sigmas[a.seed]) a.seed = c;
    p->pcg.args = a;
    if (p->pcg.trim)
        hipLaunchKernelGGL(dbslmm_pcg_init, dim3(std::max(1, p->pcg.n_prow_chip + p->pcg.n_phead)), dim3(pcg::kThreads), 0, s, a,
                           p->pcg.d_prow, p->pcg.n_prow_chip, p->pcg.n_prow - p->pcg.n_prow_chip);
    else
        hipLaunchKernelGGL(dbslmm_pcg_init, dim3(p->pcg.n_prow), dim3(pcg::kThreads), 0, s, a, p->pcg.d_prow, p->pcg.n_prow, 0);
    HIP_TRY(ctx, hipGetLastError());
    p->pcg.join = false;
    if (p->pcg.n_pflist > 0) {
        HIP_TRY(ctx, hipEventRecord(ctx->fork, s));
        HIP_TRY(ctx, hipStreamWaitEvent(ctx->stream2, ctx->fork, 0));
        if (ev) HIP_TRY(ctx, hipEventRecord(ev[kEvPcgBlockBegin], ctx->stream2));
        int grid = std::max(1, std::min(p->pcg.n_pflist, ctx->n_cu));
        if (p->opt.pcg_block_wgs > 0) grid = std::min(grid, p->opt.pcg_block_wgs);
        hipLaunchKernelGGL(dbslmm_pcg_block, dim3(grid), dim3(pcg::kThreads), pcg::block_lds_bytes(n), ctx->stream2, a,
                           p->pcg.d_pflist, p->pcg.n_pflist, p->pcg.d_pfnext, p->opt.pcg_maxit);
        HIP_TRY(ctx, hipGetLastError());
        if (ev) HIP_TRY(ctx, hipEventRecord(ev[kEvPcgBlockEnd], ctx->stream2));
        HIP_TRY(ctx, hipEventRecord(ctx->join, ctx->stream2));
        p->pcg.join = true;
    } else if (const int rc = record_instants(ctx, ev, {kEvPcgBlockBegin, kEvPcgBlockEnd}, s)) {
        return rc;
    }
    p->pcg.it = 0;
    p->pcg.pending = true;
    if (const int rc = pcg_iters(p, pcg_first_chunk(p, sigmas, n))) return rc;
    p->n_runs++;
    LastRun r;
    r.ran = true;
    r.stopped = false;
    r.sigma_run = sigmas[n - 1];
    r.var_copy = n - 1;
    r.score_copies = n;
    r.score_stale = false;
    r.pcg_ran = true;
    r.pcg_pending_var = true;
    r.cheb_base = -1;
    r.cheb_pending_var = false;
    r.cg_ran = false;
    r.cheb_iters = r.cheb_bytes = 0;
    close_run(p, r);
    return DBSLMM_OK;
}

static int stream_results(dbslmm_plan* p, double* beta_s, double* beta_l, int32_t* block_status) {
    dbslmm_ctx* ctx = p->ctx;
    const int n = p->so.n;
    const int32_t run = p->so.run;
    const double* ms = p->so.mir.get<double>();
    const double* ml = ms + static_cast<int64_t>(n) * p->n_s;
    const int32_t* mst = reinterpret_cast<const int32_t*>(ml + static_cast<int64_t>(n) * p->n_l);
    if (!p->num_block) block_status = nullptr;
    auto copy_out = [&](int b, int c) {
        const OutRange& r = p->h_orange[b];
        if (beta_s && r.s1 > r.s0)
            memcpy(beta_s + c * p->n_s + r.s0, ms + c * p->n_s + r.s0, (r.s1 - r.s0) * sizeof(double));
        if (beta_l && r.l1 > r.l0)
            memcpy(beta_l + c * p->n_l + r.l0, ml + c * p->n_l + r.l0, (r.l1 - r.l0) * sizeof(double));
        if (block_status) block_status[static_cast<int64_t>(c) * p->num_block + r.blk] = mst[c * p->nbk + r.blk];
        p->so.done[static_cast<size_t>(b) * n + c] = run;
    };
    const std::vector<int2>& pairs = p->so.h_pfpairs;
    size_t head = 0;
    bool polled = false;
    while (p->pcg.pending) {
        for (;;) {
            const hipError_t q = hipEventQuery(p->so.ev[0]);
            if (q == hipSuccess) break;
            if (q != hipErrorNotReady) HIP_TRY(ctx, q);
            polled = true;
            for (size_t e = head; e < pairs.size(); ++e) {
                const size_t f = static_cast<size_t>(pairs[e].x) * n + pairs[e].y;
                if (p->so.done[f] != run && __atomic_load_n(p->so.mflag.get<int32_t>() + f, __ATOMIC_ACQUIRE) == run)
                    copy_out(pairs[e].x, pairs[e].y);
            }
            while (head < pairs.size() && p->so.done[static_cast<size_t>(pairs[head].x) * n + pairs[head].y] == run)
                ++head;
        }
        if (const int rc = pcg_check(p)) return rc;
    }
    if (polled) (void)hipGetLastError();
    HIP_TRY(ctx, hipStreamSynchronize(ctx->stream));
    if (const int rc = check_trsv(p)) return rc;
    std::vector<CopySeg> rest;
    for (int c = 0; c < n; ++c)
        for (int b = 0; b < p->pcg.n_pblk;) {
            if (p->so.done[static_cast<size_t>(b) * n + c] == run) { ++b; continue; }
            int e = b;
            while (e + 1 < p->pcg.n_pblk && p->so.done[static_cast<size_t>(e + 1) * n + c] != run) ++e;
            const OutRange &r0 = p->h_orange[b], &r1 = p->h_orange[e];
            if (beta_s && r1.s1 > r0.s0)
                rest.push_back({beta_s + c * p->n_s + r0.s0, ms + c * p->n_s + r0.s0, (r1.s1 - r0.s0) * sizeof(double)});
            if (beta_l && r1.l1 > r0.l0)
                rest.push_back({beta_l + c * p->n_l + r0.l0, ml + c * p->n_l + r0.l0, (r1.l1 - r0.l0) * sizeof(double)});
            for (int k = b; k <= e; ++k) {
                const int32_t id = p->h_orange[k].blk;
                if (block_status) block_status[static_cast<int64_t>(c) * p->num_block + id] = mst[c * p->nbk + id];
                p->so.done[static_cast<size_t>(k) * n + c] = run;
            }
            b = e + 1;
        }
    par_memcpy_list(rest);
    for (int c = 0; c < n && block_status; ++c)
        for (int32_t b : p->h_empty) block_status[static_cast<int64_t>(c) * p->num_block + b] = DBSLMM_BLOCK_EMPTY;
    return collect_timing(p);
}
```

Measured before the change: 162.9 million.

## Move PCG convergence test into update kernel via last-arriver decision

The residual and solution norms are now accumulated during the update step rather than in the rows step. The last tile-block of each block (tracked with an atomic arrival counter) then decides convergence and marks the block done with state 4. The next update launch only writes betas and status for such blocks, which removes the rows-kernel work and one extra iteration per converged block. The fused single-block path likewise computes norms in the update loop and checks convergence at the top of the next iteration. The change adds cross-workgroup atomics and fences, and shifts iteration accounting by one, which the host-side need computation adjusts for.

```diff
diff --git a/dbslmm_amd/csrc/kernels.hip b/dbslmm_amd/csrc/kernels.hip
--- a/dbslmm_amd/csrc/kernels.hip
+++ b/dbslmm_amd/csrc/kernels.hip
@@ -193,6 +193,8 @@
     int32_t* status;
     int32_t* active;
     int32_t* next;
+    int32_t* arrive;
+    int32_t n_arrive;
 };
 extern "C" __global__ __launch_bounds__(256) void dbslmm_pcg_front(
     const v4i* __restrict__ tab, int32_t n_ref,
@@ -204,6 +206,7 @@
     if (t < f.n) f.dshift[t] = t == 0 ? f.shift[0] : t == 1 ? f.shift[1] : t == 2 ? f.shift[2] : f.shift[3];
     if (t == 0) *f.active = 0;
     if (t < 4 && f.next) f.next[t] = 0;
+    for (int i = t; i < f.n_arrive; i += nt) f.arrive[i] = 0;
     slot_stats_of(t, tab, n_ref, slot_pos, slot_block, n_slots, S_out, mu_out, rsd_out, block_flags);
 }
 
diff --git a/dbslmm_amd/csrc/pcg.hip b/dbslmm_amd/csrc/pcg.hip
--- a/dbslmm_amd/csrc/pcg.hip
+++ b/dbslmm_amd/csrc/pcg.hip
@@ -50,6 +50,8 @@
     int32_t* done;
     int32_t* active;
     int32_t* fin;
+    int32_t* arrive;
+    int32_t maxit;
     double* beta_s;
     double* beta_l;
     int32_t* status;
@@ -162,6 +164,59 @@
 }
 __device__ __forceinline__ double col_shift(const PcgArgs& a, const PcgBlk& B, int k) {
     return a.dshift[B.mshift ? a.seed : k];
+}
+
+__device__ __forceinline__ double ordered_sum_agent(const double* p, int64_t st, int s1) {
+    double acc = 0.0;
+    for (int s = 0; s < s1; s += 16) {
+        double t[16];
+#pragma unroll
+        for (int u = 0; u < 16; ++u)
+            t[u] = s + u < s1 ? __hip_atomic_load(p + static_cast<int64_t>(s + u) * st, __ATOMIC_RELAXED, __HIP_MEMORY_SCOPE_AGENT)
+                              : 0.0;
+#pragma unroll
+        for (int u = 0; u < 16; ++u) acc += t[u];
+    }
+    return acc;
+}
+
+__device__ __forceinline__ void arrive_and_decide(const PcgArgs& a, const PcgBlk& B, int bi, int lane, int it,
+                                                  const double* zeta, bool fresh) {
+    int last = 0;
+    if (lane == 0)
+        last = __hip_atomic_fetch_add(a.arrive + bi, 1, __ATOMIC_RELAXED, __HIP_MEMORY_SCOPE_AGENT) == B.Tb - 1;
+    if (!__shfl(last, 0)) return;
+    __builtin_amdgcn_fence(__ATOMIC_ACQUIRE, "wavefront");
+    if (lane == 0) __hip_atomic_store(a.arrive + bi, 0, __ATOMIC_RELAXED, __HIP_MEMORY_SCOPE_AGENT);
+    if (it >= a.maxit || __hip_atomic_load(a.done + bi, __ATOMIC_RELAXED, __HIP_MEMORY_SCOPE_AGENT) != 0) return;
+    const int n = a.ncopy, c = lane & 31;
+    double sum = 0.0;
+    if (c < n) {
+        const double* d = a.dot + B.dof;
+        sum = lane < 32 ? ordered_sum_agent(d + 2 * n + (B.mshift ? 0 : c), kNDot * n, B.Tb)
+                        : ordered_sum_agent(d + 3 * n + c, kNDot * n, B.Tb);
+    }
+    const double xx = __shfl(sum, (lane & 31) + 32);
+    bool runs = false;
+    if (lane < n) {
+        const bool was = !fresh && a.cnv[B.sco + c] != 0;
+        bool conv = was;
+        if (!was) {
+            double rr = sum;
+            double lam = a.dshift[c] + 1.0 - a.tau;
+            if (B.mshift && zeta) rr = rr * zeta[c] * zeta[c];
+            else if (B.ms != B.m) lam = 1.0 - a.tau;
+            const double t = a.tol * lam;
+            conv = rr == 0.0 || rr <= t * t * xx;
+            if (conv) __hip_atomic_store(a.cnv + B.sco + c, it + 1, __ATOMIC_RELAXED, __HIP_MEMORY_SCOPE_AGENT);
+        }
+        runs = !conv;
+    }
+    if (__ballot(runs) == 0 && lane == 0) {
+        __hip_atomic_store(a.done + bi, 4, __ATOMIC_RELAXED, __HIP_MEMORY_SCOPE_AGENT);
+        __hip_atomic_store(a.itb + bi, it + 1, __ATOMIC_RELAXED, __HIP_MEMORY_SCOPE_AGENT);
+        atomicSub(a.active, 1);
+    }
 }
 
 __device__ __forceinline__ void put_beta(const PcgArgs& a, const PcgBlk& B, int i, int k, double x, bool mono) {
@@ -382,7 +437,7 @@
 extern "C" __global__ __launch_bounds__(pcg::kThreads) void dbslmm_pcg_init(PcgArgs a, const int2* __restrict__ rows,
                                                                             int32_t n_lead, int32_t skip) {
     using namespace pcg;
-    __shared__ double red[kThreads / 64][kMaxNC];
+    __shared__ double red[kThreads / 64][kMaxNC], red2[kThreads / 64][kMaxNC];
     __shared__ int mono_s;
     const int g = blockIdx.x;
     const int2 it = rows[g < n_lead ? g : g + skip];
@@ -399,15 +454,15 @@
         if (mono) atomicOr(&mono_s, 1);
         __syncthreads();
         if (tid < n) {
-            a.cnv[B.sco + tid] = 0;
+            __hip_atomic_store(a.cnv + B.sco + tid, 0, __ATOMIC_RELAXED, __HIP_MEMORY_SCOPE_AGENT);
             double* q = a.qs + static_cast<int64_t>(B.sco + tid) * kQS;
             q[4] = q[5] = 1.0;
         }
         if (tid == 0) {
-            a.itb[bi] = 0;
+            __hip_atomic_store(a.itb + bi, 0, __ATOMIC_RELAXED, __HIP_MEMORY_SCOPE_AGENT);
             a.fin[bi] = 0;
             const bool fz = B.fused && u16;
-            a.done[bi] = mono_s ? 2 : fz ? 3 : 0;
+            __hip_atomic_store(a.done + bi, mono_s ? 2 : fz ? 3 : 0, __ATOMIC_RELAXED, __HIP_MEMORY_SCOPE_AGENT);
             if (!mono_s && !fz) atomicAdd(a.active, 1);
         }
     }
@@ -440,15 +495,36 @@
             const double rhs = a.z[B.row0 + i];
             sv[k] = a.S[B.row0 + i] * a.rsd[B.row0 + i] * (rhs / jdiag(a, B, i, col_shift(a, B, k)));
         }
-#pragma unroll
-    for (int k = 0; k < kMaxNC; ++k) sv[k] = wave_sum(sv[k]);
+    double rq[kMaxNC];
+#pragma unroll
+    for (int k = 0; k < kMaxNC; ++k) {
+        const double rhs = (k < nc && (k & 1) == h && in) ? a.z[B.row0 + i] : 0.0;
+        rq[k] = rhs * rhs;
+    }
+#pragma unroll
+    for (int k = 0; k < kMaxNC; ++k) {
+        sv[k] = wave_sum(sv[k]);
+        rq[k] = wave_sum(rq[k]);
+    }
     if ((tid & 63) == 0)
 #pragma unroll
-        for (int k = 0; k < kMaxNC; ++k) red[tid >> 6][k] = sv[k];
+        for (int k = 0; k < kMaxNC; ++k) {
+            red[tid >> 6][k] = sv[k];
+            red2[tid >> 6][k] = rq[k];
+        }
     __syncthreads();
-    if (tid < nc) {
+    if (tid < n) {
         const int hk = tid & 1;
-        a.dot[B.dof + (static_cast<int64_t>(I) * kNDot + 4) * n + tid] = red[2 * hk][tid] + red[2 * hk + 1][tid];
+        double* dt = a.dot + B.dof + static_cast<int64_t>(I) * kNDot * n + tid;
+        if (tid < nc) {
+            dt[4 * n] = red[2 * hk][tid] + red[2 * hk + 1][tid];
+            __hip_atomic_store(dt + 2 * n, red2[2 * hk][tid] + red2[2 * hk + 1][tid], __ATOMIC_RELAXED, __HIP_MEMORY_SCOPE_AGENT);
+        }
+        __hip_atomic_store(dt + 3 * n, 0.0, __ATOMIC_RELAXED, __HIP_MEMORY_SCOPE_AGENT);
+    }
+    if (tid < 64 && !(B.fused && u16)) {
+        asm volatile("s_waitcnt vmcnt(0)" ::: "memory");
+        arrive_and_decide(a, B, bi, tid, 0, nullptr, true);
     }
 }
 
@@ -478,7 +554,7 @@
 
 extern "C" __global__ __launch_bounds__(pcg::kThreads) void dbslmm_pcg_rows(PcgArgs a, const int2* __restrict__ rows) {
     using namespace pcg;
-    __shared__ double red[kThreads / 64][kMaxNC][4];
+    __shared__ double red[kThreads / 64][kMaxNC][2];
     __shared__ double sig[kMaxNC];
     chip_wide_priority();
     const int2 it = rows[blockIdx.x];
@@ -494,73 +570,85 @@
     const bool in = i < B.m;
     const double Si = in ? a.S[B.row0 + i] : 0.0, ri = in ? a.rsd[B.row0 + i] : 0.0;
     const int nrun = (I + a.run) / a.run;
-    double dv[kMaxNC][4];
+    double dv[kMaxNC][2];
+#pragma unroll
+    for (int k = 0; k < kMaxNC; ++k) dv[k][0] = dv[k][1] = 0.0;
+#pragma unroll
+    for (int k = 0; k < kMaxNC; ++k) {
+        if (k >= nc || (k & 1) != h) continue;
+        const int64_t o = k * a.vstride + B.vo + i;
+        const double* pp = a.part + B.po + static_cast<int64_t>(I) * B.Ns * nc * kT + k * kT + r;
+        double y = ordered_sum(pp, nc * kT, I, B.Tb, 0.0);
+        y = ordered_sum(pp, nc * kT, B.Tb, B.Tb + nrun, y);
+        const double dc = col_shift(a, B, k);
+        const double rv = a.R[o];
+        const double u = in ? rv / jdiag(a, B, i, dc) : 0.0;
+        const double sh = i < B.ms ? dc : 0.0;
+        double w = 0.0;
+        if (in) {
+            if (u16) w = a.tau * a.rn * ri * __builtin_fma(-Si, sig[k] * a.rn, y) + (1.0 - a.tau + sh) * u;
+            else w = y + sh * u;
+        }
+        a.W[o] = w;
+        dv[k][0] = rv * u;
+        dv[k][1] = w * u;
+    }
 #pragma unroll
     for (int k = 0; k < kMaxNC; ++k)
 #pragma unroll
-        for (int f = 0; f < 4; ++f) dv[k][f] = 0.0;
-#pragma unroll
-    for (int k = 0; k < kMaxNC; ++k) {
-        if (k >= n || (k & 1) != h) continue;
-        const int64_t o = k * a.vstride + B.vo + i;
-        if (k < nc) {
-            const double* pp = a.part + B.po + static_cast<int64_t>(I) * B.Ns * nc * kT + k * kT + r;
-            double y = ordered_sum(pp, nc * kT, I, B.Tb, 0.0);
-            y = ordered_sum(pp, nc * kT, B.Tb, B.Tb + nrun, y);
-            const double dc = col_shift(a, B, k);
-            const double rv = a.R[o];
-            const double u = in ? rv / jdiag(a, B, i, dc) : 0.0;
-            const double sh = i < B.ms ? dc : 0.0;
-            double w = 0.0;
-            if (in) {
-                if (u16) w = a.tau * a.rn * ri * __builtin_fma(-Si, sig[k] * a.rn, y) + (1.0 - a.tau + sh) * u;
-                else w = y + sh * u;
-            }
-            a.W[o] = w;
-            dv[k][0] = rv * u;
-            dv[k][1] = w * u;
-            dv[k][2] = rv * rv;
-        }
-        const double xv = a.X[o];
-        dv[k][3] = xv * xv;
-    }
-#pragma unroll
-    for (int k = 0; k < kMaxNC; ++k)
-#pragma unroll
-        for (int f = 0; f < 4; ++f) dv[k][f] = wave_sum(dv[k][f]);
+        for (int f = 0; f < 2; ++f) dv[k][f] = wave_sum(dv[k][f]);
     if ((tid & 63) == 0)
 #pragma unroll
         for (int k = 0; k < kMaxNC; ++k)
 #pragma unroll
-            for (int f = 0; f < 4; ++f) red[tid >> 6][k][f] = dv[k][f];
+            for (int f = 0; f < 2; ++f) red[tid >> 6][k][f] = dv[k][f];
     __syncthreads();
-    if (tid < 4 * n) {
-        const int k = tid >> 2, f = tid & 3, hk = k & 1;
-        if (f == 3 || k < nc)
-            a.dot[B.dof + (static_cast<int64_t>(I) * kNDot + f) * n + k] = red[2 * hk][k][f] + red[2 * hk + 1][k][f];
+    if (tid < 2 * nc) {
+        const int k = tid >> 1, f = tid & 1, hk = k & 1;
+        a.dot[B.dof + (static_cast<int64_t>(I) * kNDot + f) * n + k] = red[2 * hk][k][f] + red[2 * hk + 1][k][f];
     }
     if (I == 0 && tid == 0) a.itb[bi] += 1;
 }
 
 extern "C" __global__ __launch_bounds__(pcg::kThreads) void dbslmm_pcg_update(PcgArgs a, const int2* __restrict__ rows) {
     using namespace pcg;
-    __shared__ double tot[kMaxNC][4];
+    __shared__ double tot[kMaxNC][2];
     __shared__ double coef[kMaxNC][3];
     __shared__ double seedc[2];
+    __shared__ double zeta_s[kMaxNC];
     __shared__ int run_s[kMaxNC];
-    __shared__ double red[kThreads / 64][kMaxNC];
+    __shared__ double red[kThreads / 64][kMaxNC][3];
     chip_wide_priority();
     const int2 it = rows[blockIdx.x];
     const int bi = it.x, I = it.y, tid = threadIdx.x;
-    if (a.done[bi]) return;
+    const int done = a.done[bi];
+    if (done == 4) {
+        const PcgBlk B = a.blk[bi];
+        const int n = a.ncopy;
+        const int r = tid & (kT - 1), h = tid >> 7, i = I * kT + r;
+        if (i < B.m)
+            for (int k = h; k < n; k += 2) put_beta(a, B, i, k, a.X[k * a.vstride + B.vo + i], false);
+        if (I == 0 && tid < n) put_status(a, B, tid, false);
+        __syncthreads();
+        if (tid == 0 &&
+            __hip_atomic_fetch_add(a.fin + bi, 1, __ATOMIC_ACQ_REL, __HIP_MEMORY_SCOPE_AGENT) == B.Tb - 1) {
+            a.done[bi] = 1;
+            if (a.mir_flag)
+                for (int c = 0; c < n; ++c)
+                    __hip_atomic_store(a.mir_flag + static_cast<int64_t>(bi) * n + c, a.run_no, __ATOMIC_RELEASE,
+                                       __HIP_MEMORY_SCOPE_SYSTEM);
+        }
+        return;
+    }
+    if (done) return;
     const PcgBlk B = a.blk[bi];
     const bool u16 = on_u16(a, B);
     const int n = a.ncopy, nc = B.nc;
     const int itn = a.itb[bi] - 1;
     const int par = itn & 1;
-    if (tid < 4 * n) {
-        const int k = tid >> 2, f = tid & 3;
-        tot[k][f] = (f == 3 || k < nc) ? ordered_sum(a.dot + B.dof + f * n + k, kNDot * n, 0, B.Tb, 0.0) : 0.0;
+    if (tid < 2 * nc) {
+        const int k = tid >> 1, f = tid & 1;
+        tot[k][f] = ordered_sum(a.dot + B.dof + f * n + k, kNDot * n, 0, B.Tb, 0.0);
     }
     __syncthreads();
     if (B.mshift) {
@@ -583,18 +671,16 @@
             double* q = a.qs + static_cast<int64_t>(B.sco + c) * kQS;
             const double al = seedc[0], be = seedc[1];
             const double zk = q[4 + 2 * par], zk1 = q[4 + 2 * par + 1];
-            const double rr = tot[0][2] * zk * zk, xx = tot[c][3];
-            const double t = a.tol * (a.dshift[c] + 1.0 - a.tau);
-            const bool conv = a.cnv[B.sco + c] != 0 || rr == 0.0 || rr <= t * t * xx;
+            const bool conv = a.cnv[B.sco + c] != 0;
             const double e = a.dshift[c] - a.dshift[a.seed];
             const double cp = itn == 0 ? 0.0 : al * be / a.qs[static_cast<int64_t>(B.sco) * kQS + 2 * par + 1];
             const double zn = zk * zk1 / ((1.0 + cp + al * e) * zk1 - cp * zk);
             coef[c][0] = al * zn / zk;
             coef[c][1] = zk1 != 0.0 ? (zk / zk1) * (zk / zk1) * be : 0.0;
             coef[c][2] = zk;
+            zeta_s[c] = zn;
             run_s[c] = conv ? 0 : 1;
             if (I == 0) {
-                if (conv && a.cnv[B.sco + c] == 0) a.cnv[B.sco + c] = itn + 1;
                 q[4 + 2 * (par ^ 1)] = zn;
                 q[4 + 2 * (par ^ 1) + 1] = zk;
             }
@@ -608,10 +694,8 @@
     } else {
         if (tid < n) {
             const int k = tid;
-            const double gam = tot[k][0], del = tot[k][1], rr = tot[k][2], xx = tot[k][3];
-            const double lam = B.ms == B.m ? a.dshift[k] + 1.0 - a.tau : 1.0 - a.tau;
-            const double t = a.tol * lam;
-            const bool conv = a.cnv[B.sco + k] != 0 || rr == 0.0 || rr <= t * t * xx;
+            const double gam = tot[k][0], del = tot[k][1];
+            const bool conv = a.cnv[B.sco + k] != 0;
             double al = 0.0, be = 0.0;
             if (!conv) {
                 double* q = a.qs + static_cast<int64_t>(B.sco + k) * kQS;
@@ -625,8 +709,6 @@
                     q[2 * (par ^ 1)] = gam;
                     q[2 * (par ^ 1) + 1] = al;
                 }
-            } else if (I == 0 && a.cnv[B.sco + k] == 0) {
-                a.cnv[B.sco + k] = itn + 1;
             }
             coef[k][0] = al;
             coef[k][1] = be;
@@ -635,30 +717,11 @@
         }
         __syncthreads();
     }
-    int running = 0;
-    for (int k = 0; k < n; ++k) running += run_s[k];
-    if (running == 0) {
-        const int r = tid & (kT - 1), h = tid >> 7, i = I * kT + r;
-        if (i < B.m)
-            for (int k = h; k < n; k += 2) put_beta(a, B, i, k, a.X[k * a.vstride + B.vo + i], false);
-        if (I == 0 && tid < n) put_status(a, B, tid, false);
-        __syncthreads();
-        if (tid == 0 &&
-            __hip_atomic_fetch_add(a.fin + bi, 1, __ATOMIC_ACQ_REL, __HIP_MEMORY_SCOPE_AGENT) == B.Tb - 1) {
-            a.done[bi] = 1;
-            atomicSub(a.active, 1);
-            if (a.mir_flag)
-                for (int c = 0; c < n; ++c)
-                    __hip_atomic_store(a.mir_flag + static_cast<int64_t>(bi) * n + c, a.run_no, __ATOMIC_RELEASE,
-                                       __HIP_MEMORY_SCOPE_SYSTEM);
-        }
-        return;
-    }
     const int r = tid & (kT - 1), h = tid >> 7, i = I * kT + r;
     const bool in = i < B.m;
-    double sv[kMaxNC];
-#pragma unroll
-    for (int k = 0; k < kMaxNC; ++k) sv[k] = 0.0;
+    double sv[kMaxNC], rq[kMaxNC], xq[kMaxNC];
+#pragma unroll
+    for (int k = 0; k < kMaxNC; ++k) sv[k] = rq[k] = xq[k] = 0.0;
     if (B.mshift) {
         if (in) {
             const int64_t o0 = B.vo + i;
@@ -668,8 +731,10 @@
                 if (c >= n || (c & 1) != h || !run_s[c]) continue;
                 const int64_t o = c * a.vstride + o0;
                 const double p = __builtin_fma(coef[c][1], a.P[o], coef[c][2] * rv);
+                const double x = __builtin_fma(coef[c][0], p, a.X[o]);
                 a.P[o] = p;
-                a.X[o] = __builtin_fma(coef[c][0], p, a.X[o]);
+                a.X[o] = x;
+                xq[c] = x * x;
             }
             if (h == 0) {
                 const double al = seedc[0], be = seedc[1];
@@ -679,6 +744,7 @@
                 a.R[o0] = rn;
                 a.U[o0] = u16 ? rn * a.rsd[B.row0 + i] : rn;
                 if (u16) sv[0] = a.S[B.row0 + i] * a.rsd[B.row0 + i] * rn;
+                rq[0] = rn * rn;
             }
         }
     } else {
@@ -699,17 +765,37 @@
             a.R[o] = rn;
             a.U[o] = u16 ? (rn / dg) * a.rsd[B.row0 + i] : rn / dg;
             if (u16) sv[k] = a.S[B.row0 + i] * a.rsd[B.row0 + i] * (rn / dg);
-        }
-    }
-#pragma unroll
-    for (int k = 0; k < kMaxNC; ++k) sv[k] = wave_sum(sv[k]);
+            rq[k] = rn * rn;
+            xq[k] = x * x;
+        }
+    }
+#pragma unroll
+    for (int k = 0; k < kMaxNC; ++k) {
+        sv[k] = wave_sum(sv[k]);
+        rq[k] = wave_sum(rq[k]);
+        xq[k] = wave_sum(xq[k]);
+    }
     if ((tid & 63) == 0)
 #pragma unroll
-        for (int k = 0; k < kMaxNC; ++k) red[tid >> 6][k] = sv[k];
+        for (int k = 0; k < kMaxNC; ++k) {
+            red[tid >> 6][k][0] = sv[k];
+            red[tid >> 6][k][1] = rq[k];
+            red[tid >> 6][k][2] = xq[k];
+        }
     __syncthreads();
-    if (tid < nc && (B.mshift || run_s[tid])) {
+    if (tid < n) {
         const int hk = tid & 1;
-        a.dot[B.dof + (static_cast<int64_t>(I) * kNDot + 4) * n + tid] = red[2 * hk][tid] + red[2 * hk + 1][tid];
+        double* dt = a.dot + B.dof + static_cast<int64_t>(I) * kNDot * n + tid;
+        if (tid < nc && (B.mshift || run_s[tid])) {
+            dt[4 * n] = red[2 * hk][tid][0] + red[2 * hk + 1][tid][0];
+            __hip_atomic_store(dt + 2 * n, red[2 * hk][tid][1] + red[2 * hk + 1][tid][1], __ATOMIC_RELAXED, __HIP_MEMORY_SCOPE_AGENT);
+        }
+        if (run_s[tid])
+            __hip_atomic_store(dt + 3 * n, red[2 * hk][tid][2] + red[2 * hk + 1][tid][2], __ATOMIC_RELAXED, __HIP_MEMORY_SCOPE_AGENT);
+    }
+    if (tid < 64) {
+        asm volatile("s_waitcnt vmcnt(0)" ::: "memory");
+        arrive_and_decide(a, B, bi, tid, itn + 1, B.mshift ? zeta_s : nullptr, false);
     }
 }
 
@@ -781,7 +867,9 @@
     pcg_u4 ra[8], rb[8], rc[8];
     load(first, ra);
     load(second, rb);
-    double r[kFPer], sv[kFPer], wv[kFPer], Sr[kFPer], Rr[kFPer], sg[1] = {0.0};
+    double r[kFPer], sv[kFPer], wv[kFPer], Sr[kFPer], Rr[kFPer], sg[2 + kMaxNC];
+#pragma unroll
+    for (int k = 0; k < 2 + kMaxNC; ++k) sg[k] = 0.0;
 #pragma unroll
     for (int q = 0; q < kFPer; ++q) {
         const int i = tid + kThreads * q;
@@ -794,6 +882,7 @@
         if (in) {
             u = (r[q] / jdiag(a, B, i, dc)) * Rr[q];
             sg[0] += Sr[q] * u;
+            sg[1] = __builtin_fma(r[q], r[q], sg[1]);
         }
         Ul[i] = u;
         for (int w = 0; w < 4; ++w) yw[w * kFRows + i] = 0.0;
@@ -851,7 +940,35 @@
     }
     int it = 0;
     for (; it < maxit; ++it) {
+        if (tid == 0) {
+            const double rr = sg[1];
+            int running = 0;
+            if (msh) {
+#pragma unroll
+                for (int c = 0; c < kMaxNC; ++c) {
+                    if (c >= n) continue;
+                    const double zk = st[4 + c];
+                    const double t = a.tol * (a.dshift[c] + 1.0 - a.tau);
+                    const double rrc = rr * zk * zk;
+                    if (!flag[c] && (rrc == 0.0 || rrc <= t * t * sg[2 + c])) {
+                        flag[c] = 1;
+                        a.cnv[B.sco + c] = it + 1;
+                    }
+                    running += flag[c] ? 0 : 1;
+                }
+            } else {
+                const double lam = B.ms == B.m ? dc + 1.0 - a.tau : 1.0 - a.tau;
+                const double t = a.tol * lam;
+                if (rr == 0.0 || rr <= t * t * sg[2]) {
+                    flag[0] = 1;
+                    a.cnv[B.sco + cc] = it + 1;
+                }
+                running = flag[0] ? 0 : 1;
+            }
+            flag[kMaxNC] = running;
+        }
         __syncthreads();
+        if (flag[kMaxNC] == 0) break;
         {
             QPos pm = first, pl = second;
             adv(pl, 4);
@@ -885,9 +1002,7 @@
             }
         }
         __syncthreads();
-        double d[3 + kMaxNC];
-#pragma unroll
-        for (int k = 0; k < 3 + kMaxNC; ++k) d[k] = 0.0;
+        double d[2] = {0.0, 0.0};
 #pragma unroll
         for (int q = 0; q < kFPer; ++q) {
             const int i = tid + kThreads * q;
@@ -905,16 +1020,11 @@
                 wv[q] = w;
                 d[0] += r[q] * u;
                 d[1] += w * u;
-                d[2] += r[q] * r[q];
-                for (int c = 0; c < nx; ++c) {
-                    const double xv = Xl[c * kFRows + i];
-                    d[3 + c] += xv * xv;
-                }
             }
         }
         block_sum(d, red, tid);
         if (tid == 0) {
-            const double gam = d[0], del = d[1], rr = d[2];
+            const double gam = d[0], del = d[1];
             double al, be = 0.0;
             if (it == 0) {
                 al = gam / del;
@@ -922,17 +1032,10 @@
                 be = gam / st[0];
                 al = gam / (del - be * gam / st[1]);
             }
-            int running = 0;
             if (msh) {
                 const double cp = it == 0 ? 0.0 : al * be / st[1];
                 for (int c = 0; c < n; ++c) {
                     const double zk = st[4 + c], zk1 = st[8 + c];
-                    const double t = a.tol * (a.dshift[c] + 1.0 - a.tau);
-                    const double rrc = rr * zk * zk;
-                    if (!flag[c] && (rrc == 0.0 || rrc <= t * t * d[3 + c])) {
-                        flag[c] = 1;
-                        a.cnv[B.sco + c] = it + 1;
-                    }
                     const double e = a.dshift[c] - a.dshift[a.seed];
                     const double zn = zk * zk1 / ((1.0 + cp + al * e) * zk1 - cp * zk);
                     st[12 + 3 * c] = al * zn / zk;
@@ -940,27 +1043,17 @@
                     st[12 + 3 * c + 2] = zk;
                     st[8 + c] = zk;
                     st[4 + c] = zn;
-                    running += flag[c] ? 0 : 1;
                 }
-            } else {
-                const double lam = B.ms == B.m ? dc + 1.0 - a.tau : 1.0 - a.tau;
-                const double t = a.tol * lam;
-                if (rr == 0.0 || rr <= t * t * d[3]) {
-                    flag[0] = 1;
-                    a.cnv[B.sco + cc] = it + 1;
-                }
-                running = flag[0] ? 0 : 1;
             }
             st[0] = gam;
             st[1] = al;
             st[2] = al;
             st[3] = be;
-            flag[kMaxNC] = running;
         }
         __syncthreads();
-        if (flag[kMaxNC] == 0) break;
         const double al = st[2], be = st[3];
-        double sg2[1] = {0.0};
+#pragma unroll
+        for (int k = 0; k < 2 + kMaxNC; ++k) sg[k] = 0.0;
 #pragma unroll
         for (int q = 0; q < kFPer; ++q) {
             const int i = tid + kThreads * q;
@@ -980,22 +1073,31 @@
                 sv[q] = sn;
                 r[q] = rn;
                 Ul[i] = rn * rsd_i;
+#pragma unroll
+                for (int c = 0; c < kMaxNC; ++c) {
+                    if (c >= n) continue;
+                    const double xv = Xl[c * kFRows + i];
+                    sg[2 + c] = __builtin_fma(xv, xv, sg[2 + c]);
+                }
             } else {
                 const double dg = jdiag(a, B, i, dc);
                 const double u = r[q] / dg;
                 const double pv = __builtin_fma(be, Pl[i], u);
                 const double sn = __builtin_fma(be, sv[q], wv[q]);
+                const double xv = __builtin_fma(al, pv, Xl[i]);
                 Pl[i] = pv;
-                Xl[i] = __builtin_fma(al, pv, Xl[i]);
+                Xl[i] = xv;
                 rn = __builtin_fma(-al, sn, r[q]);
                 sv[q] = sn;
                 r[q] = rn;
                 Ul[i] = (rn / dg) * rsd_i;
-            }
-            sg2[0] += Sr[q] * Ul[i];
-        }
-        block_sum(sg2, red, tid);
-        sig = sg2[0];
+                sg[2] = __builtin_fma(xv, xv, sg[2]);
+            }
+            sg[0] += Sr[q] * Ul[i];
+            sg[1] = __builtin_fma(rn, rn, sg[1]);
+        }
+        block_sum(sg, red, tid);
+        sig = sg[0];
     }
 #pragma unroll
     for (int q = 0; q < kFPer; ++q) {
diff --git a/dbslmm_amd/csrc/plan_state.hpp b/dbslmm_amd/csrc/plan_state.hpp
--- a/dbslmm_amd/csrc/plan_state.hpp
+++ b/dbslmm_amd/csrc/plan_state.hpp
@@ -123,6 +123,7 @@
     bool join = false;
     double *d_pvec = nullptr, *d_ppart = nullptr, *d_pdot = nullptr, *d_pqs = nullptr;
     int32_t *d_pcnv = nullptr, *d_pitb = nullptr, *d_pdone = nullptr, *d_pact = nullptr, *d_pfin = nullptr;
+    int32_t* d_parr = nullptr;
     int64_t vstride = 0;
     PinnedBuf mon;
     int32_t it = 0;
diff --git a/dbslmm_amd/csrc/route_pcg.hip b/dbslmm_amd/csrc/route_pcg.hip
--- a/dbslmm_amd/csrc/route_pcg.hip
+++ b/dbslmm_amd/csrc/route_pcg.hip
@@ -35,7 +35,7 @@
     HIP_TRY(ctx, hipStreamSynchronize(ctx->stream));
     DevBufs& B = p->bufs;
     B.release_all(p->pcg.d_pblk, p->pcg.d_pitem, p->pcg.d_prow, p->pcg.d_pvec, p->pcg.d_ppart, p->pcg.d_pdot, p->pcg.d_pqs, p->pcg.d_pcnv,
-                  p->pcg.d_pitb, p->pcg.d_pdone, p->pcg.d_pact, p->pcg.d_pflist, p->pcg.d_pfin);
+                  p->pcg.d_pitb, p->pcg.d_pdone, p->pcg.d_pact, p->pcg.d_pflist, p->pcg.d_pfin, p->pcg.d_parr);
     p->pcg.n = 0;
     p->pcg.trim = false;
     using namespace pcg;
@@ -120,6 +120,7 @@
     HIP_TRY(ctx, B.alloc(&p->pcg.d_pdone, p->pcg.n_pblk));
     HIP_TRY(ctx, B.alloc(&p->pcg.d_pact, 1));
     HIP_TRY(ctx, B.alloc(&p->pcg.d_pfin, p->pcg.n_pblk));
+    HIP_TRY(ctx, B.alloc(&p->pcg.d_parr, p->pcg.n_pblk));
     p->pcg.n = n;
     return DBSLMM_OK;
 }
@@ -172,7 +173,7 @@
         HIP_TRY(ctx, hipStreamSynchronize(ctx->stream));
         int32_t need = 0;
         for (int b = 0; b < p->pcg.n_pblk; ++b)
-            if (p->pcg.h_pfused.empty() || !p->pcg.h_pfused[b]) need = std::max(need, p->pcg.h_mon()[1 + b]);
+            if (p->pcg.h_pfused.empty() || !p->pcg.h_pfused[b]) need = std::max(need, p->pcg.h_mon()[1 + b] - 1);
         if (p->pcg.h_mon()[0] <= 0 || p->pcg.it >= p->opt.pcg_maxit) {
             p->pcg.pending = false;
             p->pcg.need = p->pcg.h_mon()[0] <= 0 ? need : p->opt.pcg_maxit;
@@ -267,6 +268,8 @@
     fr.status = p->d_status;
     fr.active = p->pcg.d_pact;
     fr.next = p->pcg.n_pflist > 0 ? p->pcg.d_pfnext : nullptr;
+    fr.arrive = p->pcg.d_parr;
+    fr.n_arrive = p->pcg.n_pblk;
     hipLaunchKernelGGL(dbslmm_pcg_front, dim3(std::max(1, (p->n_slots + 255) / 256)), dim3(256), 0, s, p->img.rows(),
                        p->n_ref, p->d_slot_pos, p->d_slot_block, p->n_slots, p->d_S, p->d_mu, p->d_rsd, p->d_flags, fr);
     HIP_TRY(ctx, hipGetLastError());
@@ -304,6 +307,8 @@
     a.done = p->pcg.d_pdone;
     a.active = p->pcg.d_pact;
     a.fin = p->pcg.d_pfin;
+    a.arrive = p->pcg.d_parr;
+    a.maxit = p->opt.pcg_maxit;
     a.beta_s = p->d_beta_s;
     a.beta_l = p->d_beta_l;
     a.status = p->d_status;
```

After: 163.3 million (median of 3 runs). Within noise of the previous version (+0.2%).
